# moxime/joint-vae

Hardware: AMD Instinct MI355X
Metric: training_images_per_sec (higher is better)
Workload: dtype f32

## Files before the change

include/jvae_hip.h:

```cpp
#ifndef JVAE_HIP_H
#define JVAE_HIP_H

#include <stddef.h>

#ifdef __cplusplus
extern "C" {
#endif

const char* jvae_version(void);

int jvae_gemm_f32(int M, int N, int K, int batch,
                  const float* A, long sAm, long sAk, long sAb,
                  const float* B, long sBk, long sBn, long sBb,
                  float* C, long sCm, long sCn, long sCb,
                  const float* bias, int bias_mode, int flags, int splitk, void* stream);

int jvae_splitk_fold_f32(const float* part, const float* bias, float* y, int S, long MN, int N, int relu, int accumulate,
                         void* stream);

size_t jvae_conv2d_workspace_bytes(int N, int Cin, int H, int W, int Cout, int KH, int KW, int S, int P, int OP,
                                   int transposed);
int jvae_conv2d_set_split_bf16(int mode);
int jvae_conv2d_set_split_shape16(int on);
int jvae_conv2d_out_shape(int H, int W, int KH, int KW, int S, int P, int OP, int transposed, int* OH, int* OW);
int jvae_conv2d_route(int dir, int layout, int bias, int stats, int y_f32, int aff_kind,
                      int N, int Cin, int H, int W, int Cout, int KH, int KW, int S, int P, int OP, int transposed,
                      int* kernel, int* swap, size_t* ws_bytes, int* splits, int* aff_ok);
const char* jvae_conv2d_kernel_name(int kernel);
int jvae_conv2d_fwd_f32(const float* x, const float* w, const float* bias, float* y,
                        int N, int Cin, int H, int W, int Cout, int KH, int KW, int S, int P, int OP, int transposed,
                        void* ws, size_t ws_bytes, void* stream);
int jvae_conv2d_stats_splits(int N, int Cin, int H, int W, int Cout, int KH, int KW, int S, int P, int OP, int transposed);
int jvae_conv2d_fwd_stats_f32(const float* x, const float* w, const float* bias, float* y, float* stats, int* nsplit,
                              int N, int Cin, int H, int W, int Cout, int KH, int KW, int S, int P, int OP, int transposed,
                              void* ws, size_t ws_bytes, void* stream);
int jvae_conv2d_dgrad_f32(const float* dy, const float* w, float* dx,
                          int N, int Cin, int H, int W, int Cout, int KH, int KW, int S, int P, int OP, int transposed,
                          void* ws, size_t ws_bytes, void* stream);
int jvae_conv2d_wgrad_f32(const float* x, const float* dy, float* dw, float* dbias, int accumulate,
                          int N, int Cin, int H, int W, int Cout, int KH, int KW, int S, int P, int OP, int transposed,
                          void* ws, size_t ws_bytes, void* stream);

int jvae_pack_cache_configure(void* buf, size_t bytes);
int jvae_pack_cache_begin(void* stream, long long owner, const void* const* weights, int n);
int jvae_pack_cache_end(void);
int jvae_pack_cache_pin(void);
int jvae_pack_cache_reset(void);
int jvae_pack_cache_stats(int* entries, long long* hits, long long* misses, long long* refreshes);

size_t jvae_channel_sum_workspace_bytes(int C);
int jvae_channel_sum_f32(const float* t, float* out, int N, int C, int P, int accumulate, void* ws, size_t ws_bytes,
                         void* stream);

size_t jvae_bn_workspace_bytes(int C);
int jvae_bn_plan(int N, int C, int P, int* nsplit, int* nchunk);
int jvae_image_range(int N, int parts, int j, int* nb, int* ne);
int jvae_bn_fwd_f32(const float* x, const float* gamma, const float* beta,
                    float* running_mean, float* running_var, long long* num_batches_tracked,
                    float* y, float* save_mean, float* save_invstd,
                    int N, int C, int P, float momentum, float eps, int training, int relu,
                    void* ws, size_t ws_bytes, void* stream);
int jvae_bn_fwd_ext_f32(const float* x, const float* gamma, const float* beta,
                        float* running_mean, float* running_var, long long* num_batches_tracked,
                        float* y, float* save_mean, float* save_invstd,
                        int N, int C, int P, float momentum, float eps, int training, int relu,
                        const float* ext_stats, int ext_nsplit, const float* ext_pivot,
                        void* ws, size_t ws_bytes, void* stream);
int jvae_bn_bwd_f32(const float* dy, const float* x, const float* gamma, const float* beta,
                    const float* save_mean, const float* save_invstd,
                    float* dx, float* dgamma, float* dbeta, int accumulate,
                    int N, int C, int P, int relu, void* ws, size_t ws_bytes, void* stream);
int jvae_bn_eval_bwd_f32(const float* dy, const float* x, const float* gamma, const float* beta,
                         const float* running_mean, const float* running_var, float* dx,
                         int N, int C, int P, float eps, int relu, void* stream);

int jvae_bn_finalize_f32(const float* x, const float* gamma, const float* beta,
                         float* running_mean, float* running_var, long long* num_batches_tracked,
                         float* save_mean, float* save_invstd, float* scale, float* shift,
                         int N, int C, int P, float momentum, float eps, int training,
                         const float* ext_stats, int ext_nsplit, const float* ext_pivot,
                         void* ws, size_t ws_bytes, void* stream);
int jvae_conv2d_affine_ok(int N, int Cin, int H, int W, int Cout, int KH, int KW, int S, int P, int OP, int transposed);
int jvae_conv2d_fwd_aff_f32(const float* x, const float* w, const float* bias, float* y, float* stats, int* nsplit,
                            const float* in_scale, const float* in_shift, int in_relu,
                            int N, int Cin, int H, int W, int Cout, int KH, int KW, int S, int P, int OP, int transposed,
                            void* ws, size_t ws_bytes, void* stream);
int jvae_conv2d_wgrad_aff_f32(const float* x, const float* dy, float* dw, float* dbias, int accumulate,
                              const float* in_scale, const float* in_shift, int in_relu,
                              int N, int Cin, int H, int W, int Cout, int KH, int KW, int S, int P, int OP, int transposed,
                              void* ws, size_t ws_bytes, void* stream);

int jvae_bn_sums_f32(const float* x, const float* pivot, float* sums, int N, int C, int P,
                     void* ws, size_t ws_bytes, void* stream);
int jvae_bn_fwd_sync_f32(const float* x, const float* gamma, const float* beta,
                         float* running_mean, float* running_var, long long* num_batches_tracked,
                         float* y, float* save_mean, float* save_invstd,
                         int N, int C, int P, float momentum, float eps, int relu,
                         const float* global_sums, const float* pivot, int world,
                         void* ws, size_t ws_bytes, void* stream);
int jvae_bn_bwd_sums_f32(const float* dy, const float* x, const float* gamma, const float* beta,
                         const float* save_mean, const float* save_invstd, float* local_sums,
                         int N, int C, int P, int relu, void* ws, size_t ws_bytes, void* stream);
int jvae_bn_bwd_sync_f32(const float* dy, const float* x, const float* gamma, const float* beta,
                         const float* save_mean, const float* save_invstd,
                         const float* local_sums, const float* global_sums, int world,
                         float* dx, float* dgamma, float* dbeta, int accumulate,
                         int N, int C, int P, int relu, void* stream);

int jvae_b8_pack_f32(const float* x, void* y, int N, int C, long HW, void* stream);
int jvae_b8_unpack_f32(const void* y, float* x, int N, int C, long HW, int accumulate, void* stream);
int jvae_conv2d_native_b8(int N, int Cin, int H, int W, int Cout, int KH, int KW, int S, int P, int OP, int transposed);
size_t jvae_conv2d_workspace_bytes_b8(int N, int Cin, int H, int W, int Cout, int KH, int KW, int S, int P, int OP,
                                      int transposed);
int jvae_conv2d_stats_splits_b8(int N, int Cin, int H, int W, int Cout, int KH, int KW, int S, int P, int OP, int transposed);
int jvae_conv2d_fwd_b8(const void* x, const float* w, const float* bias, void* y, int y_f32, float* stats, int* nsplit,
                       int N, int Cin, int H, int W, int Cout, int KH, int KW, int S, int P, int OP, int transposed,
                       void* ws, size_t ws_bytes, void* stream);
int jvae_conv2d_dgrad_b8(const void* dy, const float* w, void* dx,
                         int N, int Cin, int H, int W, int Cout, int KH, int KW, int S, int P, int OP, int transposed,
                         void* ws, size_t ws_bytes, void* stream);
int jvae_conv2d_wgrad_b8(const void* x, const void* dy, float* dw, float* dbias, int accumulate,
                         int N, int Cin, int H, int W, int Cout, int KH, int KW, int S, int P, int OP, int transposed,
                         void* ws, size_t ws_bytes, void* stream);
size_t jvae_bn_workspace_bytes_b8(int C);
int jvae_bn_plan_b8(int N, int C, long HW, int* nsplit, int* nchunk);
int jvae_bn_fwd_b8(const void* x, const float* gamma, const float* beta,
                   float* running_mean, float* running_var, long long* num_batches_tracked,
                   void* y, float* save_mean, float* save_invstd,
                   int N, int C, long HW, float momentum, float eps, int training, int relu,
                   const float* ext_stats, int ext_nsplit, const float* ext_pivot,
                   void* ws, size_t ws_bytes, void* stream);
int jvae_bn_bwd_b8(const void* dy, const void* x, const float* gamma, const float* beta,
                   const float* save_mean, const float* save_invstd,
                   void* dx, float* dgamma, float* dbeta, int accumulate,
                   int N, int C, long HW, int relu, void* ws, size_t ws_bytes, void* stream);
int jvae_bn_finalize_b8(const void* x, const float* gamma, const float* beta,
                        float* running_mean, float* running_var, long long* num_batches_tracked,
                        float* save_mean, float* save_invstd, float* coef,
                        int N, int C, long HW, float momentum, float eps, int training,
                        const float* ext_stats, int ext_nsplit, const float* ext_pivot,
                        void* ws, size_t ws_bytes, void* stream);
int jvae_bn_sums_b8(const void* x, const float* pivot, float* sums, int N, int C, long HW,
                    void* ws, size_t ws_bytes, void* stream);
int jvae_bn_fwd_sync_b8(const void* x, const float* gamma, const float* beta,
                        float* running_mean, float* running_var, long long* num_batches_tracked,
                        void* y, float* save_mean, float* save_invstd,
                        int N, int C, long HW, float momentum, float eps, int relu,
                        const float* global_sums, const float* pivot, int world,
                        void* ws, size_t ws_bytes, void* stream);
int jvae_bn_bwd_sums_b8(const void* dy, const void* x, const float* gamma, const float* beta,
                        const float* save_mean, const float* save_invstd, float* local_sums,
                        int N, int C, long HW, int relu, void* ws, size_t ws_bytes, void* stream);
int jvae_bn_bwd_sync_b8(const void* dy, const void* x, const float* gamma, const float* beta,
                        const float* save_mean, const float* save_invstd,
                        const float* local_sums, const float* global_sums, int world,
                        void* dx, float* dgamma, float* dbeta, int accumulate,
                        int N, int C, long HW, int relu, void* ws, size_t ws_bytes, void* stream);
int jvae_conv2d_affine_ok_b8(int N, int Cin, int H, int W, int Cout, int KH, int KW, int S, int P, int OP, int transposed);
int jvae_conv2d_fwd_aff_b8(const void* x, const float* w, const float* bias, void* y, int y_f32, float* stats, int* nsplit,
                           const float* in_scale, const float* in_shift, int in_relu,
                           int N, int Cin, int H, int W, int Cout, int KH, int KW, int S, int P, int OP, int transposed,
                           void* ws, size_t ws_bytes, void* stream);
int jvae_conv2d_wgrad_aff_b8(const void* x, const void* dy, float* dw, float* dbias, int accumulate,
                             const float* in_scale, const float* in_shift, int in_relu,
                             int N, int Cin, int H, int W, int Cout, int KH, int KW, int S, int P, int OP, int transposed,
                             void* ws, size_t ws_bytes, void* stream);
int jvae_relu_fwd_b8(const void* x, void* y, long units, void* stream);
int jvae_relu_bwd_b8(const void* dy, const void* y, void* dx, long units, void* stream);

int jvae_act_fwd_f32(const float* x, float* y, long n, int kind, void* stream);
int jvae_act_bwd_f32(const float* dy, const float* y, float* dx, long n, int kind, void* stream);

int jvae_dict_stats_f32(const float* means, float* dict, int C, int K, void* stream);
int jvae_latent_fwd_f32(const float* mu, const float* lv_raw, const float* eps, const long long* y,
                        const float* means, const float* T, const float* dict,
                        float* lv, float* z, float* kl, float* zdist, float* var_kl, float* dzdist,
                        int N, int K, int L, int C, int prior, int var_dim, float tau, float alpha, float w,
                        int sampled, int has_forced, float forced_lv, void* stream);
int jvae_latent_bwd_f32(const float* mu, const float* lv_raw, const float* lv, const float* eps, const long long* y,
                        const float* means, const float* T,
                        const float* gz, const float* g_kl, const float* g_zdist, const float* g_vkl,
                        const float* gmu_direct, const float* glv_direct,
                        float* gmu, float* glv_raw, float* gmeans, float* gT,
                        int N, int K, int L, int C, int prior, int var_dim, float tau, float alpha, float w,
                        int sampled, int has_forced, void* ws, size_t ws_bytes, void* stream);
int jvae_latent_fwd_wdev_f32(const float* mu, const float* lv_raw, const float* eps, const long long* y,
                             const float* means, const float* T, const float* dict,
                             float* lv, float* z, float* kl, float* zdist, float* var_kl, float* dzdist,
                             int N, int K, int L, int C, int prior, int var_dim, float tau, float alpha, float w,
                             int sampled, int has_forced, float forced_lv, const float* w_dev, void* stream);
int jvae_latent_bwd_wdev_f32(const float* mu, const float* lv_raw, const float* lv, const float* eps, const long long* y,
                             const float* means, const float* T,
                             const float* gz, const float* g_kl, const float* g_zdist, const float* g_vkl,
                             const float* gmu_direct, const float* glv_direct,
                             float* gmu, float* glv_raw, float* gmeans, float* gT,
                             int N, int K, int L, int C, int prior, int var_dim, float tau, float alpha, float w,
                             int sampled, int has_forced, const float* w_dev, void* ws, size_t ws_bytes, void* stream);

int jvae_recon_fwd_f32(const float* x_reco, const float* x, const float* sigma, int sigma_is_log,
                       float* wmse, int L, int N, int D, void* stream);
int jvae_recon_bwd_f32(const float* x_reco, const float* x, const float* sigma, int sigma_is_log, const float* sigma_fwd,
                       const float* g_wmse, const float* wmse, float* g_x_reco, float* gsigma, int accumulate_sigma,
                       int L, int N, int D, void* ws, size_t ws_bytes, void* stream);

int jvae_mse_rows_fwd_f32(const float* rows, const float* x, float* wmse, int L, int N, int D, void* stream);
int jvae_mse_rows_bwd_f32(const float* rows, const float* x, const float* g_wmse, float* g_rows, int L, int N, int D, void* stream);

int jvae_elbo_fwd_f32(const float* wmse_s, const float* kl, const float* ce, const float* sigma, int sigma_is_log,
                      float* wmse, float* cross_x, float* total, float* mse, int L, int N, int D, float beta, float cw,
                      void* stream);
int jvae_elbo_bwd_f32(const float* g_wmse, const float* g_cx, const float* g_tot, const float* sigma, int sigma_is_log,
                      float* g_wmse_s, float* g_kl, float* g_ce, float* gsigma, int accumulate_sigma,
                      int L, int N, int D, float beta, float cw, void* ws, size_t ws_bytes, void* stream);
int jvae_elbo_fwd_wdev_f32(const float* wmse_s, const float* kl, const float* ce, const float* sigma, int sigma_is_log,
                           float* wmse, float* cross_x, float* total, float* mse, int L, int N, int D, float beta, float cw,
                           const float* cw_dev, void* stream);
int jvae_elbo_bwd_wdev_f32(const float* g_wmse, const float* g_cx, const float* g_tot, const float* sigma, int sigma_is_log,
                           float* g_wmse_s, float* g_kl, float* g_ce, float* gsigma, int accumulate_sigma,
                           int L, int N, int D, float beta, float cw, const float* cw_dev, void* ws, size_t ws_bytes,
                           void* stream);

int jvae_dropout_f32(const float* x, float* y, long n, float p, long seed, void* stream);
int jvae_dropout_dev_f32(const float* x, float* y, long n, float p, const long long* seed_dev, long salt, void* stream);

int jvae_iws_f32(const float* wmse_s, const float* eps, const float* log_var, const float* log_pz, const float* sigma,
                 int sigma_is_log, int L, int N, int K, int C, int D, float* rows, float* iws, void* stream);

int jvae_measures_f32(const float* sumsq_x, long nx, const float* wmse, const float* zdist, const float* var_kl, int N, int Nz,
                      const float* sigma, int sigma_is_log, const float* means, int C, int K, const int* flag,
                      const float* prev, int batch, float* out, void* stream);
int jvae_measures_dev_f32(const float* sumsq_x, long nx, const float* wmse, const float* zdist, const float* var_kl, int N, int Nz,
                          const float* sigma, int sigma_is_log, const float* means, int C, int K, const int* flag,
                          float* run, int* counter, void* stream);

int jvae_loss_sums_f32(const float* const* rows, const long* lens, int nrows, float* acc, void* stream);

int jvae_xent_fwd_f32(const float* logits, const long long* y, float* ce, int R, int N, int C, void* stream);
int jvae_xent_bwd_f32(const float* logits, const long long* y, const float* g_ce, float* g_logits, int R, int N, int C,
                      void* stream);

size_t jvae_sqnorm_workspace_bytes(void);
int jvae_sqnorm_accum_f32(const float* g, long n, float* acc, int reset, void* ws, size_t ws_bytes, void* stream);
int jvae_clip_scale_f32(float* g, long n, const float* sqnorm, float max_norm, void* stream);
int jvae_adam_step_f32(float* p, const float* g, float* m, float* v, long n,
                       float lr, float beta1, float beta2, float eps, float weight_decay, long step,
                       float max_norm, const float* sqnorm, int* nonfinite_flag, void* stream);
int jvae_adam_step_dev_f32(float* p, const float* g, float* m, float* v, long n, float* hyper, int advance,
                           float eps, float weight_decay, float max_norm, const float* sqnorm, int* nonfinite_flag,
                           void* stream);

int jvae_sgd_step_f32(float* p, const float* g, float* buf, long n, float lr, float momentum, int nesterov,
                      float weight_decay, int first_step, float max_norm, const float* sqnorm, int* nonfinite_flag,
                      void* stream);

int jvae_pool2d_out_shape(int H, int W, int K, int S, int P, int* OH, int* OW);
int jvae_pool2d_fwd_f32(const float* x, float* y, int* idx, long planes, int H, int W, int K, int S, int P, int mode,
                        void* stream);
int jvae_pool2d_bwd_f32(const float* dy, const int* idx, float* dx, long planes, int H, int W, int K, int S, int P,
                        int mode, void* stream);
int jvae_upsample_nearest_fwd_f32(const float* x, float* y, long planes, int H, int W, int scale, void* stream);
int jvae_upsample_nearest_bwd_f32(const float* dy, float* dx, long planes, int H, int W, int scale, void* stream);
int jvae_pool2d_fwd_b8(const void* x, void* y, int* idx, long blocks, int H, int W, int K, int S, int P, int mode, void* stream);
int jvae_pool2d_bwd_b8(const void* dy, const int* idx, void* dx, long blocks, int H, int W, int K, int S, int P, int mode,
                       void* stream);
int jvae_upsample_nearest_fwd_b8(const void* x, void* y, long blocks, int H, int W, int scale, void* stream);
int jvae_upsample_nearest_bwd_b8(const void* dy, void* dx, long blocks, int H, int W, int scale, void* stream);

int jvae_augment_u8_f32(const unsigned char* in, const unsigned char* flip, const int* dy, const int* dx,
                        float* out, int N, int C, int H, int W, int pad, int nhwc, void* stream);

size_t jvae_roc_workspace_bytes(int M, long n_in, long n_out);
int jvae_roc_curve_f32(const float* ins, const float* outs, const double* kept_tpr, const int* two_sided,
                       double* auc, double* kept_fpr, double* kept_tpr_out, double* thr_low, double* thr_up, int* status,
                       int M, long n_in, long n_out, int K, void* ws, size_t ws_bytes, void* stream);

int jvae_misclass_scores_f32(const float* src, const int* kinds, const float* temps, const int* rows, float* out,
                             int R, int C, long N, long out_stride, void* stream);
size_t jvae_misclass_split_workspace_bytes(long N);
int jvae_misclass_split_f32(const float* scores, const unsigned char* mask, float* out, int* n_correct, int M, long N,
                            void* ws, size_t ws_bytes, void* stream);
int jvae_misclass_confusion_f32(const float* scores, const unsigned char* mask, const double* thr, int* tp, int* fp,
                                int M, long N, int K, void* stream);

int jvae_odin_head_f32(const float* logits, const float* temps, float* scores, float* dlogits,
                       int F, int L, int N, int C, long stride_f, long stride_l, void* stream);
int jvae_odin_perturb_f32(float* acc, const float* g, const float* x, const float* eps, float* out, long numel, int E,
                          void* stream);

#ifdef __cplusplus
}
#endif
#endif
```

joint-vae_amd/csrc/conv_api.hip:

```cpp
#include "common.h"
#include "jvae_internal.h"
#include "conv_dispatch.h"

namespace {

inline ConvRoute route(const ConvGeom& g, int transposed, ConvDir dir, CallFlags f = {}) {
    return jvae_conv_route(g, transposed, dir, CONV_F32, f);
}

bool affine_ok(const ConvGeom& g, int transposed, ConvDir other, const ConvRoute& r) {
    return r.aff_ok && route(g, transposed, other, {false, false, false, 1}).aff_ok;
}

int fwd_f32(const float* x, const float* w, const float* bias, float* y, float* stats, int* nsplit, const InAff* aff,
            int N, int Cin, int H, int W, int Cout, int KH, int KW, int S, int P, int OP, int transposed,
            void* ws, size_t ws_bytes, void* stream) {
    ConvGeom g; int oh, ow;
    if (nsplit) *nsplit = 0;
    if (!jvae_make_geom(N, Cin, H, W, Cout, KH, KW, S, P, OP, transposed, &g, &oh, &ow)) return JVAE_EINVAL;
    const ConvRoute r = route(g, transposed, CONV_FWD, {bias != nullptr, stats != nullptr, false, jvae_aff_kind(aff)});
    if (aff && !affine_ok(g, transposed, CONV_WGRAD, r)) return JVAE_ENOTSUP;
    if (N == 0) return 0;
    if (jvae_ws_short(r, ws, ws_bytes)) return JVAE_EWORKSPACE;
    return jvae_conv_run_fwd(r, g, x, w, bias, y, (float*)ws, ws_bytes, (hipStream_t)stream, stats, nsplit, aff);
}

int wgrad_f32(const float* x, const float* dy, float* dw, float* dbias, int accumulate, const InAff* aff,
              int N, int Cin, int H, int W, int Cout, int KH, int KW, int S, int P, int OP, int transposed,
              void* ws, size_t ws_bytes, void* stream) {
    ConvGeom g; int oh, ow;
    if (!dw || (N > 0 && (!x || !dy))) return JVAE_EINVAL;
    if (!jvae_make_geom(N, Cin, H, W, Cout, KH, KW, S, P, OP, transposed, &g, &oh, &ow)) return JVAE_EINVAL;
    const ConvRoute r = route(g, transposed, CONV_WGRAD, {false, false, false, jvae_aff_kind(aff)});
    if (aff && !affine_ok(g, transposed, CONV_FWD, r)) return JVAE_ENOTSUP;
    if (N > 0 && jvae_ws_short(r, ws, ws_bytes)) return JVAE_EWORKSPACE;
    hipStream_t st = (hipStream_t)stream;
    if (!accumulate) {
        hipError_t e = hipMemsetAsync(dw, 0, sizeof(float) * (size_t)Cin * Cout * KH * KW, st);
        if (e != hipSuccess) return (int)e;
    }
    if (N == 0) {
        if (dbias && !accumulate) {
            hipError_t e = hipMemsetAsync(dbias, 0, sizeof(float) * (size_t)Cout, st);
            if (e != hipSuccess) return (int)e;
        }
        return 0;
    }
    int rc = jvae_conv_run_wgrad(r, g, transposed, x, dy, dw, (float*)ws, ws_bytes, st, aff);
    if (rc) return rc;
    if (dbias) rc = jvae_channel_sum(dy, dbias, N, Cout, oh * ow, accumulate, (float*)ws, ws_bytes, st);
    return rc;
}

}

extern "C" {

int jvae_conv2d_set_split_bf16(int mode) { return jvae_conv5_x3_set(mode); }
int jvae_conv2d_set_split_shape16(int on) { return jvae_conv5_x3_set_shape16(on); }

size_t jvae_conv2d_workspace_bytes(int N, int Cin, int H, int W, int Cout, int KH, int KW, int S, int P, int OP,
                                   int transposed) {
    ConvGeom g; int oh, ow;
    if (!jvae_make_geom(N, Cin, H, W, Cout, KH, KW, S, P, OP, transposed, &g, &oh, &ow)) return 0;
    return jvae_conv_ws(g, transposed);
}

int jvae_conv2d_route(int dir, int layout, int bias, int stats, int y_f32, int aff_kind,
                      int N, int Cin, int H, int W, int Cout, int KH, int KW, int S, int P, int OP, int transposed,
                      int* kernel, int* swap, size_t* ws_bytes, int* splits, int* aff_ok) {
    ConvGeom g; int oh, ow;
    if (dir != CONV_FWD && dir != CONV_DGRAD && dir != CONV_WGRAD) return JVAE_EINVAL;
    if ((layout != CONV_F32 && layout != CONV_B8) || aff_kind < 0 || aff_kind > 2) return JVAE_EINVAL;
    if (!jvae_make_geom(N, Cin, H, W, Cout, KH, KW, S, P, OP, transposed, &g, &oh, &ow)) return JVAE_EINVAL;
    const ConvRoute r = jvae_conv_route(g, transposed, (ConvDir)dir, (ConvLayout)layout,
                                        {bias != 0, stats != 0, y_f32 != 0, aff_kind});
    if (kernel) *kernel = (int)r.k;
    if (swap) *swap = r.swap ? 1 : 0;
    if (ws_bytes) *ws_bytes = r.ws;
    if (splits) *splits = r.splits;
    if (aff_ok) *aff_ok = r.aff_ok ? 1 : 0;
    return 0;
}

const char* jvae_conv2d_kernel_name(int kernel) {
    switch (kernel) {
#define JVAE_CK_NAME(k) case k: return #k;
        JVAE_CK_NAME(CK_NONE) JVAE_CK_NAME(CK_GENERIC) JVAE_CK_NAME(CK_POINT) JVAE_CK_NAME(CK_SMALLCO)
        JVAE_CK_NAME(CK_SMALLCI) JVAE_CK_NAME(CK_FWD5) JVAE_CK_NAME(CK_FWD5_X3) JVAE_CK_NAME(CK_T2) JVAE_CK_NAME(CK_T2_X3)
        JVAE_CK_NAME(CK_WG5) JVAE_CK_NAME(CK_WG5_X3) JVAE_CK_NAME(CK_B8) JVAE_CK_NAME(CK_T2_B8) JVAE_CK_NAME(CK_WG_B8)
        JVAE_CK_NAME(CK_WG_B8X) JVAE_CK_NAME(CK_SMALLCO_DG)
#undef JVAE_CK_NAME
        default: return nullptr;
    }
}

int jvae_conv2d_out_shape(int H, int W, int KH, int KW, int S, int P, int OP, int transposed, int* OH, int* OW) {
    ConvGeom g;
    if (!OH || !OW) return JVAE_EINVAL;
    return jvae_make_geom(1, 1, H, W, 1, KH, KW, S, P, OP, transposed, &g, OH, OW) ? 0 : JVAE_EINVAL;
}

int jvae_conv2d_fwd_f32(const float* x, const float* w, const float* bias, float* y,
                        int N, int Cin, int H, int W, int Cout, int KH, int KW, int S, int P, int OP, int transposed,
                        void* ws, size_t ws_bytes, void* stream) {
    if (!w || (N > 0 && (!x || !y))) return JVAE_EINVAL;
    return fwd_f32(x, w, bias, y, nullptr, nullptr, nullptr, N, Cin, H, W, Cout, KH, KW, S, P, OP, transposed, ws, ws_bytes,
                   stream);
}

int jvae_conv2d_stats_splits(int N, int Cin, int H, int W, int Cout, int KH, int KW, int S, int P, int OP, int transposed) {
    ConvGeom g; int oh, ow;
    if (!jvae_make_geom(N, Cin, H, W, Cout, KH, KW, S, P, OP, transposed, &g, &oh, &ow)) return 0;
    return route(g, transposed, CONV_FWD, {false, true, false, 0}).splits;
}

int jvae_conv2d_fwd_stats_f32(const float* x, const float* w, const float* bias, float* y, float* stats, int* nsplit,
                              int N, int Cin, int H, int W, int Cout, int KH, int KW, int S, int P, int OP, int transposed,
                              void* ws, size_t ws_bytes, void* stream) {
    if (!w || !nsplit || (N > 0 && (!x || !y))) return JVAE_EINVAL;
    return fwd_f32(x, w, bias, y, stats, nsplit, nullptr, N, Cin, H, W, Cout, KH, KW, S, P, OP, transposed, ws, ws_bytes, stream);
}

int jvae_conv2d_affine_ok(int N, int Cin, int H, int W, int Cout, int KH, int KW, int S, int P, int OP, int transposed) {
    ConvGeom g; int oh, ow;
    if (!jvae_make_geom(N, Cin, H, W, Cout, KH, KW, S, P, OP, transposed, &g, &oh, &ow)) return 0;
    return affine_ok(g, transposed, CONV_WGRAD, route(g, transposed, CONV_FWD, {false, false, false, 1})) ? 1 : 0;
}

int jvae_conv2d_fwd_aff_f32(const float* x, const float* w, const float* bias, float* y, float* stats, int* nsplit,
                            const float* in_scale, const float* in_shift, int in_relu,
                            int N, int Cin, int H, int W, int Cout, int KH, int KW, int S, int P, int OP, int transposed,
                            void* ws, size_t ws_bytes, void* stream) {
    if (!w || !in_scale || !in_shift || (N > 0 && (!x || !y))) return JVAE_EINVAL;
    if (stats && !nsplit) return JVAE_EINVAL;
    const InAff aff{in_scale, in_shift, in_relu};
    return fwd_f32(x, w, bias, y, stats, nsplit, &aff, N, Cin, H, W, Cout, KH, KW, S, P, OP, transposed, ws, ws_bytes, stream);
}

int jvae_conv2d_wgrad_aff_f32(const float* x, const float* dy, float* dw, float* dbias, int accumulate,
                              const float* in_scale, const float* in_shift, int in_relu,
                              int N, int Cin, int H, int W, int Cout, int KH, int KW, int S, int P, int OP, int transposed,
                              void* ws, size_t ws_bytes, void* stream) {
    if (!in_scale || !in_shift) return JVAE_EINVAL;
    const InAff aff{in_scale, in_shift, in_relu};
    return wgrad_f32(x, dy, dw, dbias, accumulate, &aff, N, Cin, H, W, Cout, KH, KW, S, P, OP, transposed, ws, ws_bytes, stream);
}

int jvae_conv2d_dgrad_f32(const float* dy, const float* w, float* dx,
                          int N, int Cin, int H, int W, int Cout, int KH, int KW, int S, int P, int OP, int transposed,
                          void* ws, size_t ws_bytes, void* stream) {
    ConvGeom g; int oh, ow;
    if (!w || (N > 0 && (!dy || !dx))) return JVAE_EINVAL;
    if (!jvae_make_geom(N, Cin, H, W, Cout, KH, KW, S, P, OP, transposed, &g, &oh, &ow)) return JVAE_EINVAL;
    if (N == 0) return 0;
    const ConvRoute r = route(g, transposed, CONV_DGRAD);
    if (jvae_ws_short(r, ws, ws_bytes)) return JVAE_EWORKSPACE;
    return jvae_conv_run_fwd(r, g, dy, w, nullptr, dx, (float*)ws, ws_bytes, (hipStream_t)stream);
}

int jvae_conv2d_wgrad_f32(const float* x, const float* dy, float* dw, float* dbias, int accumulate,
                          int N, int Cin, int H, int W, int Cout, int KH, int KW, int S, int P, int OP, int transposed,
                          void* ws, size_t ws_bytes, void* stream) {
    return wgrad_f32(x, dy, dw, dbias, accumulate, nullptr, N, Cin, H, W, Cout, KH, KW, S, P, OP, transposed, ws, ws_bytes, stream);
}

size_t jvae_channel_sum_workspace_bytes(int C) { return jvae_channel_sum_ws_bytes(C); }

int jvae_channel_sum_f32(const float* t, float* out, int N, int C, int P, int accumulate, void* ws, size_t ws_bytes,
                         void* stream) {
    if (!t || !out || N < 0 || C <= 0 || P <= 0) return JVAE_EINVAL;
    return jvae_channel_sum(t, out, N, C, P, accumulate, (float*)ws, ws_bytes, (hipStream_t)stream);
}

}
```

joint-vae_amd/csrc/conv_dispatch.h:

```cpp
#pragma once
#include "common.h"
#include "jvae_internal.h"

size_t jvae_conv_generic_ws(const ConvGeom& g);
int jvae_fold_fwd(const ConvGeom& g, const float* xb, const float* w, const float* bias, float* ys,
                  float* ws, size_t ws_bytes, hipStream_t st);
int jvae_fold_bwd(const ConvGeom& g, const float* ys, const float* w, const float* bias, float* xb,
                  float* ws, size_t ws_bytes, hipStream_t st);
int jvae_fold_wgrad(const ConvGeom& g, const float* xb, const float* ys, float* dw,
                    float* ws, size_t ws_bytes, hipStream_t st);
size_t jvae_channel_sum_ws_bytes(int C);
int jvae_channel_sum(const float* t, float* out, int N, int C, int P, int accumulate, float* ws, size_t ws_bytes,
                     hipStream_t st);

bool jvae_conv5_fwd_ok(int Cin, int H, int W, int Cout, int OH, int OW, int S, int P);
size_t jvae_conv5_pack_floats(int Cin, int Cout);
int jvae_conv5_fwd(const float* in, const float* w, int swap, int flip, const float* bias, float* out,
                   int N, int Cin, int H, int W, int Cout, int OW, int S, int P, float* ws, hipStream_t st,
                   float* stats = nullptr, int* nsplit = nullptr, const InAff* aff = nullptr);
int jvae_conv5_fwd_max_splits(int N, int OW);

int jvae_conv5_pack(const float* w, float* wp, int C, int O, int swap, int flip, hipStream_t st);

bool jvae_conv5_x3_ok(int Cin, int H, int W, int Cout, int OH, int OW, int S, int P);
size_t jvae_conv5_x3_pack_bytes(int Cin, int Cout);
int jvae_conv5_x3_set(int mode);
int jvae_conv5_x3_set_shape16(int on);
bool jvae_conv5_x3_enabled();
int jvae_conv5_x3_wpack(const float* w, float* ws, int C, int O, int swap, int flip, hipStream_t st);
bool jvae_convt2_x3_ok(int N, int C, int WS, int O);
int jvae_convt2_x3(const float* in, const float* w, const float* bias, float* out, int N, int C, int WS, int O, float* ws,
                   hipStream_t st, float* stats = nullptr, int* nsplit = nullptr, const InAff* aff = nullptr);
int jvae_conv5_x3_fwd(const float* in, const float* w, int swap, int flip, const float* bias, float* out,
                      int N, int Cin, int H, int W, int Cout, int OW, int S, int P, float* ws, hipStream_t st,
                      float* stats = nullptr, int* nsplit = nullptr, const InAff* aff = nullptr);

bool jvae_convt2_ok(int C, int HS, int WS, int O, int HB, int WB, int KH, int KW, int S, int P);
int jvae_convt2(const float* in, const float* wpacked, const float* bias, float* out, int N, int C, int WS, int O,
                hipStream_t st, float* stats = nullptr, int* nsplit = nullptr, const InAff* aff = nullptr);

bool jvae_conv5_smallco_ok(int Cin, int H, int W, int Cout, int KH, int KW, int S, int P);
int jvae_conv5_smallco(const float* in, const float* w, const float* bias, float* out, int N, int Cin, int W, int Cout,
                       hipStream_t st, const InAff* aff = nullptr);
int jvae_conv5_smallco_dgrad(const float* dy, const float* w, float* dx, int N, int Cy, int W, int Cx, hipStream_t st);

bool jvae_conv5_smallci_ok(int Cin, int H, int W, int Cout, int OW, int S, int P, bool dgrad_role);
int jvae_conv5_smallci(const float* in, const float* w, int swap, int flip, const float* bias, float* out,
                       int N, int Cin, int W, int Cout, float* ws, hipStream_t st, float* stats = nullptr, int* nsplit = nullptr);

bool jvae_conv5_wgrad_ok(int Ca, int HS, int WS, int Cb, int HB, int WB, int S, int P);
size_t jvae_conv5_wgrad_ws_floats(int N, int Ca, int Cb, int S, int WS);
int jvae_conv5_wgrad(const float* ps, const float* q, float* dw, int accumulate, int swapflip,
                     int N, int Ca, int WS, int Cb, int S, int P, float* ws, hipStream_t st,
                     const InAff* aff_p = nullptr, const InAff* aff_q = nullptr);

bool jvae_conv5_wgrad_x3_ok(int Ca, int HS, int WS, int Cb, int HB, int WB, int S, int P);
size_t jvae_conv5_wgrad_x3_ws_floats(int N, int Ca, int Cb, int S);
int jvae_conv5_wgrad_x3(const float* ps, const float* q, float* dw, int accumulate, int swapflip,
                        int N, int Ca, int WS, int Cb, int S, int P, float* ws, hipStream_t st,
                        const InAff* aff_p = nullptr, const InAff* aff_q = nullptr);

bool jvae_make_geom(int N, int Cin, int H, int W, int Cout, int KH, int KW, int S, int P, int OP, int transposed,
                    ConvGeom* g, int* OH, int* OW);

enum ConvDir { CONV_FWD = 1, CONV_DGRAD = 2, CONV_WGRAD = 4 };
enum ConvLayout { CONV_F32, CONV_B8 };
enum ConvKernel {
    CK_NONE,
    CK_GENERIC, CK_POINT,
    CK_SMALLCO, CK_SMALLCI, CK_FWD5, CK_FWD5_X3, CK_T2, CK_T2_X3, CK_WG5, CK_WG5_X3,
    CK_B8, CK_T2_B8, CK_WG_B8, CK_WG_B8X,
    CK_SMALLCO_DG,
};
struct CallFlags {
    bool bias, stats;
    bool y_f32;
    int aff;
};
struct ConvRoute {
    ConvKernel k;
    bool swap;
    int S, P;
    size_t ws;
    int splits;
    bool aff_ok;
};
ConvRoute jvae_conv_route(const ConvGeom& g, int transposed, ConvDir dir, ConvLayout layout, CallFlags f);
inline int jvae_aff_kind(const InAff* aff) { return !aff ? 0 : (aff->relu == JVAE_ACT_LEAKY ? 2 : 1); }
inline bool jvae_ws_short(const ConvRoute& r, const void* ws, size_t ws_bytes) { return r.ws && (!ws || ws_bytes < r.ws); }
template <class T>
inline void jvae_wgrad_operands(const ConvRoute& r, int transposed, T* x, T* dy, const InAff* aff, T** ps, T** q,
                                const InAff** aff_p, const InAff** aff_q) {
    const bool p_is_x = r.swap != (transposed != 0);
    *ps = p_is_x ? x : dy;
    *q = p_is_x ? dy : x;
    *aff_p = p_is_x ? aff : nullptr;
    *aff_q = p_is_x ? nullptr : aff;
}

size_t jvae_conv_ws(const ConvGeom& g, int transposed);
int jvae_conv_run_fwd(const ConvRoute& r, const ConvGeom& g, const float* in, const float* w, const float* bias, float* out,
                      float* ws, size_t ws_bytes, hipStream_t st, float* stats = nullptr, int* nsplit = nullptr,
                      const InAff* aff = nullptr);
int jvae_conv_run_wgrad(const ConvRoute& r, const ConvGeom& g, int transposed, const float* x, const float* dy, float* dw,
                        float* ws, size_t ws_bytes, hipStream_t st, const InAff* aff = nullptr);
```

joint-vae_amd/csrc/conv_dispatch.hip:

```cpp
#include "common.h"
#include "conv_dispatch.h"
#include "conv_b8.h"
#include "pack_elems.h"

namespace {

inline bool is5(const ConvGeom& g) { return g.KH == 5 && g.KW == 5; }
inline bool is3p1(const ConvGeom& g) { return g.KH == 3 && g.KW == 3 && g.P == 1; }
inline size_t max_sz(size_t a, size_t b) { return a > b ? a : b; }

inline bool point_input(const ConvGeom& g) {
    return g.Hs == 1 && g.Ws == 1 && g.P == 0 && g.S == 1 && g.Hb == g.KH && g.Wb == g.KW;
}
inline int point_wgrad_pieces(const ConvGeom& g) {
    const int want = (int)(1024 / ((long)cdiv(g.Cs, 64) * cdiv(g.Cb * g.KH * g.KW, 64)));
    return want < 1 ? 1 : (want > 8 ? 8 : want);
}

struct FwdOp { int Ci, H, W, Co, OH, OW; };
inline FwdOp fwd_op(const ConvGeom& g, bool small_in) {
    return small_in ? FwdOp{g.Cs, g.Hs, g.Ws, g.Cb, g.Hb, g.Wb} : FwdOp{g.Cb, g.Hb, g.Wb, g.Cs, g.Hs, g.Ws};
}
struct WgOp { int Ca, HS, WS, Cb, HB, WB; };
inline WgOp wg_op(const ConvGeom& g, bool swap) {
    return swap ? WgOp{g.Cb, g.Hb, g.Wb, g.Cs, g.Hs, g.Ws} : WgOp{g.Cs, g.Hs, g.Ws, g.Cb, g.Hb, g.Wb};
}

inline bool b8_aff_ok(int Cin, const CallFlags& f) { return (Cin + 7) / 8 * 8 <= 256 && f.aff != 2; }

ConvRoute fwd_route(const ConvGeom& g, int transposed, ConvDir dir, bool b8, const CallFlags& f) {
    const bool small_in = (dir == CONV_FWD) == (transposed != 0);
    const FwdOp o = fwd_op(g, small_in);
    ConvRoute r{CK_NONE, small_in, small_in ? 1 : g.S, small_in ? g.KH - 1 - g.P : g.P, 0, 0, false};
    if (!b8 && transposed && point_input(g)) {
        r.k = CK_POINT;
        if (!small_in) r.ws = 4 * (size_t)16 * g.N * g.Cs;
        return r;
    }
    if (!b8 && dir == CONV_FWD && !transposed && jvae_conv5_smallco_ok(g.Cb, g.Hb, g.Wb, g.Cs, g.KH, g.KW, g.S, g.P)) {
        r.k = CK_SMALLCO;
        r.aff_ok = g.Cb <= 256;
        return r;
    }
    if (!b8 && dir == CONV_DGRAD && !transposed && g.Hs == g.Hb && g.Ws == g.Wb &&
        jvae_conv5_smallco_ok(g.Cs, g.Hb, g.Wb, g.Cb, g.KH, g.KW, g.S, g.P)) {
        r.k = CK_SMALLCO_DG;
        return r;
    }
    if (small_in && g.S == 2) {
        if (b8 && jvae_convt2_b8_ok(g.Cs, g.Hs, g.Ws, g.Cb, g.Hb, g.Wb, g.KH, g.KW, g.S, g.P) && !f.y_f32) {
            r = ConvRoute{CK_T2_B8, true, 2, g.P, jvae_conv5_b8_pack_bytes(g.Cs, g.Cb, g.KH), jvae_conv5_b8_max_splits(g.N, g.Ws),
                          b8_aff_ok(g.Cs, f)};
        } else if (!b8 && jvae_convt2_ok(g.Cs, g.Hs, g.Ws, g.Cb, g.Hb, g.Wb, g.KH, g.KW, g.S, g.P)) {
            r = ConvRoute{jvae_convt2_x3_ok(g.N, g.Cs, g.Ws, g.Cb) ? CK_T2_X3 : CK_T2, true, 2, g.P,
                          4 * jvae_conv5_pack_floats(g.Cs, g.Cb), jvae_conv5_fwd_max_splits(g.N, g.Ws), true};
        }
    } else if ((is5(g) || (b8 && is3p1(g))) && (!small_in || g.S == 1)) {
        if (b8 && jvae_conv5_b8_fwd_ok(o.Ci, o.H, o.W, o.Co, o.OH, o.OW, r.S, r.P, g.KH)) {
            r.k = CK_B8;
            r.ws = jvae_conv5_b8_pack_bytes(o.Ci, o.Co, g.KH);
            r.splits = jvae_conv5_b8_max_splits(g.N, o.OW);
            r.aff_ok = b8_aff_ok(o.Ci, f);
        } else if (!b8 && jvae_conv5_fwd_ok(o.Ci, o.H, o.W, o.Co, o.OH, o.OW, r.S, r.P)) {
            if (jvae_conv5_x3_ok(o.Ci, o.H, o.W, o.Co, o.OW, o.OW, r.S, r.P)) r.k = CK_FWD5_X3;
            else if (!f.aff && jvae_conv5_smallci_ok(o.Ci, o.H, o.W, o.Co, o.OW, r.S, r.P, !f.bias && !f.stats)) r.k = CK_SMALLCI;
            else r.k = CK_FWD5;
            r.ws = 4 * jvae_conv5_pack_floats(o.Ci, o.Co);
            r.splits = jvae_conv5_fwd_max_splits(g.N, o.OW);
            r.aff_ok = true;
        }
    }
    if (r.k == CK_NONE && !b8) r = ConvRoute{CK_GENERIC, small_in, g.S, g.P, 0, 0, false};
    return r;
}

ConvRoute wgrad_route(const ConvGeom& g, int transposed, bool b8, const CallFlags& f) {
    const int few = b8 ? 8 : 15;
    const bool swap = g.S == 1 && g.Cs <= few && g.Cb > few && g.Hs == g.Hb;
    const WgOp o = wg_op(g, swap);
    ConvRoute r{CK_NONE, swap, swap ? 1 : g.S, swap ? g.KH - 1 - g.P : g.P, 0, 0, false};
    if ((is5(g) || is3p1(g)) && b8 && jvae_conv5_wgrad_b8_ok(o.Ca, o.HS, o.WS, o.Cb, o.HB, o.WB, r.S, r.P, g.KH)) {
        const bool x = is5(g) && jvae_conv5_wgrad_b8x_ok(o.Ca, o.WS, o.WS, o.Cb, o.WS * r.S, o.WS * r.S, r.S, r.P);
        r.k = x ? CK_WG_B8X : CK_WG_B8;
        r.ws = 4 * jvae_conv5_wgrad_b8_ws_floats(g.N, o.Ca, o.Cb, g.KH);
        r.aff_ok = f.aff != 2;
    } else if (is5(g) && !b8 && jvae_conv5_wgrad_ok(o.Ca, o.HS, o.WS, o.Cb, o.HB, o.WB, r.S, r.P)) {
        const bool x = jvae_conv5_wgrad_x3_ok(o.Ca, o.WS, o.WS, o.Cb, o.WS * r.S, o.WS * r.S, r.S, r.P);
        r.k = x ? CK_WG5_X3 : CK_WG5;
        r.ws = 4 * jvae_conv5_wgrad_ws_floats(g.N, o.Ca, o.Cb, r.S, o.WS);
        r.aff_ok = true;
    } else if (!b8 && transposed && point_input(g)) {
        r.k = CK_POINT;
        r.ws = 4 * (size_t)point_wgrad_pieces(g) * g.Cs * g.Cb * g.KH * g.KW;
    } else if (!b8) {
        r.k = CK_GENERIC;
    }
    return r;
}

inline const float* packed_f32(const float* w, float* ws, int C, int O, int swap, int flip, hipStream_t st) {
    bool fresh = true;
    float* slot = (float*)jvae_pack_cache_get(JVAE_PACK_F32, w, C, O, swap, flip, &fresh);
    if (slot && fresh) return slot;
    float* dst = slot ? slot : ws;
    return jvae_conv5_pack(w, dst, C, O, swap, flip, st) == 0 ? dst : nullptr;
}

}

bool jvae_make_geom(int N, int Cin, int H, int W, int Cout, int KH, int KW, int S, int P, int OP, int transposed,
                    ConvGeom* g, int* OH, int* OW) {
    if (N < 0 || Cin <= 0 || Cout <= 0 || H <= 0 || W <= 0 || KH <= 0 || KW <= 0 || S <= 0 || P < 0 || OP < 0)
        return false;
    g->N = N; g->KH = KH; g->KW = KW; g->S = S; g->P = P;
    if (!transposed) {
        if (OP != 0) return false;
        *OH = (H + 2 * P - KH) / S + 1;
        *OW = (W + 2 * P - KW) / S + 1;
        g->Cb = Cin; g->Hb = H; g->Wb = W;
        g->Cs = Cout; g->Hs = *OH; g->Ws = *OW;
    } else {
        if (OP >= S && OP != 0) return false;
        *OH = (H - 1) * S - 2 * P + KH + OP;
        *OW = (W - 1) * S - 2 * P + KW + OP;
        g->Cs = Cin; g->Hs = H; g->Ws = W;
        g->Cb = Cout; g->Hb = *OH; g->Wb = *OW;
    }
    return *OH > 0 && *OW > 0;
}

ConvRoute jvae_conv_route(const ConvGeom& g, int transposed, ConvDir dir, ConvLayout layout, CallFlags f) {
    if (dir == CONV_WGRAD) return wgrad_route(g, transposed, layout == CONV_B8, f);
    return fwd_route(g, transposed, dir, layout == CONV_B8, f);
}

size_t jvae_conv_ws(const ConvGeom& g, int transposed) {
    size_t a = max_sz(jvae_conv_generic_ws(g), jvae_channel_sum_ws_bytes(g.Cb > g.Cs ? g.Cb : g.Cs));
    for (ConvDir d : {CONV_FWD, CONV_DGRAD, CONV_WGRAD}) a = max_sz(a, jvae_conv_route(g, transposed, d, CONV_F32, {}).ws);
    if (is5(g)) a = max_sz(a, 4 * jvae_conv5_pack_floats(g.Cb, g.Cs));
    if (transposed && point_input(g)) a = max_sz(a, 4 * (size_t)8 * g.Cs * g.Cb * g.KH * g.KW);
    return a;
}

int jvae_conv_run_fwd(const ConvRoute& r, const ConvGeom& g, const float* in, const float* w, const float* bias, float* out,
                      float* ws, size_t ws_bytes, hipStream_t st, float* stats, int* nsplit, const InAff* aff) {
    const FwdOp o = fwd_op(g, r.swap);
    const int sw = r.swap ? 1 : 0;
    switch (r.k) {
        case CK_SMALLCO: return jvae_conv5_smallco(in, w, bias, out, g.N, g.Cb, g.Wb, g.Cs, st, aff);
        case CK_SMALLCO_DG: return jvae_conv5_smallco_dgrad(in, w, out, g.N, g.Cs, g.Wb, g.Cb, st);
        case CK_SMALLCI: return jvae_conv5_smallci(in, w, sw, sw, bias, out, g.N, o.Ci, o.W, o.Co, ws, st, stats, nsplit);
        case CK_FWD5_X3:
            return jvae_conv5_x3_fwd(in, w, sw, sw, bias, out, g.N, o.Ci, o.H, o.W, o.Co, o.OW, r.S, r.P, ws, st, stats, nsplit, aff);
        case CK_FWD5:
            return jvae_conv5_fwd(in, w, sw, sw, bias, out, g.N, o.Ci, o.H, o.W, o.Co, o.OW, r.S, r.P, ws, st, stats, nsplit, aff);
        case CK_T2_X3: return jvae_convt2_x3(in, w, bias, out, g.N, g.Cs, g.Ws, g.Cb, ws, st, stats, nsplit, aff);
        case CK_T2: {
            const float* wp = packed_f32(w, ws, g.Cs, g.Cb, 1, 0, st);
            if (!wp) return JVAE_EINVAL;
            return jvae_convt2(in, wp, bias, out, g.N, g.Cs, g.Ws, g.Cb, st, stats, nsplit, aff);
        }
        case CK_POINT: {
            const int cols = g.Cb * g.KH * g.KW;
            if (r.swap)
                return jvae_gemm_launch_ex(g.N, cols, g.Cs, 1, in, g.Cs, 1, 0, w, cols, 1, 0, out, cols, 1, 0,
                                           bias, bias ? 1 : 0, g.KH * g.KW, 0, 1, st);
            const long outf = (long)g.N * g.Cs;
            int S = 0;
            int rc = jvae_gemm_launch_part(g.N, g.Cs, cols, 1, in, cols, 1, 0, w, 1, cols, 0, ws, g.Cs, 1, 0, outf, 16, &S, st);
            if (rc) return rc;
            return jvae_splitk_fold(ws, nullptr, out, S, outf, g.Cs, 0, 0, st);
        }
        case CK_GENERIC:
            return r.swap ? jvae_fold_bwd(g, in, w, bias, out, ws, ws_bytes, st) : jvae_fold_fwd(g, in, w, bias, out, ws, ws_bytes, st);
        default: return JVAE_ENOTSUP;
    }
}

int jvae_conv_run_wgrad(const ConvRoute& r, const ConvGeom& g, int transposed, const float* x, const float* dy, float* dw,
                        float* ws, size_t ws_bytes, hipStream_t st, const InAff* aff) {
    const float *ps, *q;
    const InAff *aff_p, *aff_q;
    jvae_wgrad_operands(r, transposed, x, dy, aff, &ps, &q, &aff_p, &aff_q);
    const WgOp o = wg_op(g, r.swap);
    const float* big = transposed ? dy : x;
    const float* small = transposed ? x : dy;
    switch (r.k) {
        case CK_WG5_X3:
            return jvae_conv5_wgrad_x3(ps, q, dw, 1, r.swap, g.N, o.Ca, o.WS, o.Cb, r.S, r.P, ws, st,
                                       aff_p, aff_q);
        case CK_WG5:
            return jvae_conv5_wgrad(ps, q, dw, 1, r.swap, g.N, o.Ca, o.WS, o.Cb, r.S, r.P, ws, st,
                                    aff_p, aff_q);
        case CK_POINT: {
            const int cols = g.Cb * g.KH * g.KW;
            const long outf = (long)g.Cs * cols;
            int S = 0;
            int rc = jvae_gemm_launch_part(g.Cs, cols, g.N, 1, small, 1, g.Cs, 0, big, cols, 1, 0, ws, cols, 1, 0, outf,
                                           point_wgrad_pieces(g), &S, st);
            if (rc) return rc;
            return jvae_splitk_fold(ws, nullptr, dw, S, outf, cols, 0, 1, st);
        }
        case CK_GENERIC: return jvae_fold_wgrad(g, big, small, dw, ws, ws_bytes, st);
        default: return JVAE_ENOTSUP;
    }
}
```

joint-vae_amd/csrc/conv_generic.hip:

```cpp
#include "common.h"
#include "jvae_internal.h"

namespace {

__global__ __launch_bounds__(256) void unfold_kernel(const float* __restrict__ xb, float* __restrict__ col,
                                                     ConvGeom g, int n0, int nimg, long sn, long sk, long sq,
                                                     int kfast) {
    const int Kd = g.Cb * g.KH * g.KW, Ps = g.Hs * g.Ws;
    const long total = (long)nimg * Kd * Ps;
    for (long i = (long)blockIdx.x * blockDim.x + threadIdx.x; i < total; i += (long)gridDim.x * blockDim.x) {
        int n, k, q;
        if (kfast) { k = (int)(i % Kd); long r = i / Kd; n = (int)(r % nimg); q = (int)(r / nimg); }
        else       { q = (int)(i % Ps); long r = i / Ps; k = (int)(r % Kd);  n = (int)(r / Kd); }
        const int kw = k % g.KW, kh = (k / g.KW) % g.KH, cb = k / (g.KW * g.KH);
        const int hs = q / g.Ws, ws = q % g.Ws;
        const int hb = hs * g.S + kh - g.P, wb = ws * g.S + kw - g.P;
        float v = 0.f;
        if (hb >= 0 && hb < g.Hb && wb >= 0 && wb < g.Wb)
            v = xb[(((long)(n0 + n) * g.Cb + cb) * g.Hb + hb) * g.Wb + wb];
        col[(long)n * sn + (long)k * sk + (long)q * sq] = v;
    }
}

template <bool KFAST>
__global__ __launch_bounds__(256) void unfold4_kernel(const float* __restrict__ xb, float* __restrict__ col,
                                                      ConvGeom g, int n0, int nimg) {
    const unsigned Kd = g.Cb * g.KH * g.KW, Ps = g.Hs * g.Ws, KK = g.KH * g.KW;
    const unsigned inner4 = (KFAST ? Kd : Ps) / 4;
    const unsigned total = (KFAST ? Ps * (unsigned)nimg : (unsigned)nimg * Kd) * inner4;
    for (unsigned i = blockIdx.x * blockDim.x + threadIdx.x; i < total; i += gridDim.x * blockDim.x) {
        const unsigned row = i / inner4, e4 = (i - row * inner4) * 4;
        unsigned n, k, q;
        if (KFAST) { q = row / nimg; n = row - q * nimg; k = e4; }
        else       { n = row / Kd;   k = row - n * Kd;   q = e4; }
        unsigned cb = k / KK, t = k - cb * KK;
        unsigned kh = t / g.KW, kw = t - kh * g.KW;
        const unsigned hs = q / g.Ws, ws = q - hs * g.Ws;
        const float* src = xb + (long)(n0 + n) * g.Cb * g.Hb * g.Wb;
        f32x4 v;
#pragma unroll
        for (int e = 0; e < 4; ++e) {
            const int hb = (int)(hs * g.S + kh) - g.P;
            const int wb = (int)((KFAST ? ws : ws + e) * g.S + kw) - g.P;
            v[e] = (hb >= 0 && hb < g.Hb && wb >= 0 && wb < g.Wb) ? src[((long)cb * g.Hb + hb) * g.Wb + wb] : 0.f;
            if (KFAST && ++kw == (unsigned)g.KW) { kw = 0; if (++kh == (unsigned)g.KH) { kh = 0; ++cb; } }
        }
        *reinterpret_cast<f32x4*>(col + (long)i * 4) = v;
    }
}

__global__ __launch_bounds__(256) void fold_kernel(const float* __restrict__ col, float* __restrict__ xb,
                                                   const float* __restrict__ bias, ConvGeom g, int n0, int nimg,
                                                   long sn, long sk, long sq) {
    const unsigned total = (unsigned)nimg * g.Cb * g.Hb * g.Wb;
    for (unsigned i = blockIdx.x * blockDim.x + threadIdx.x; i < total; i += gridDim.x * blockDim.x) {
        unsigned r = i / (unsigned)g.Wb;
        const int wb = (int)(i - r * g.Wb);
        unsigned r2 = r / (unsigned)g.Hb;
        const int hb = (int)(r - r2 * g.Hb);
        const int n = (int)(r2 / (unsigned)g.Cb);
        const int cb = (int)(r2 - (unsigned)n * g.Cb);
        float acc = bias ? bias[cb] : 0.f;
        if (g.Hs * g.Ws < g.KH * g.KW) {
            for (int hs = 0; hs < g.Hs; ++hs) {
                const int kh = hb + g.P - hs * g.S;
                if (kh < 0 || kh >= g.KH) continue;
                for (int ws = 0; ws < g.Ws; ++ws) {
                    const int kw = wb + g.P - ws * g.S;
                    if (kw < 0 || kw >= g.KW) continue;
                    const int k = (cb * g.KH + kh) * g.KW + kw;
                    acc += col[(long)n * sn + (long)k * sk + (long)(hs * g.Ws + ws) * sq];
                }
            }
            xb[(((long)(n0 + n) * g.Cb + cb) * g.Hb + hb) * g.Wb + wb] = acc;
            continue;
        }
        for (int kh = 0; kh < g.KH; ++kh) {
            const int th = hb + g.P - kh;
            if (th < 0 || th % g.S) continue;
            const int hs = th / g.S;
            if (hs >= g.Hs) continue;
            for (int kw = 0; kw < g.KW; ++kw) {
                const int tw = wb + g.P - kw;
                if (tw < 0 || tw % g.S) continue;
                const int ws = tw / g.S;
                if (ws >= g.Ws) continue;
                const int k = (cb * g.KH + kh) * g.KW + kw;
                acc += col[(long)n * sn + (long)k * sk + (long)(hs * g.Ws + ws) * sq];
            }
        }
        xb[(((long)(n0 + n) * g.Cb + cb) * g.Hb + hb) * g.Wb + wb] = acc;
    }
}

__global__ __launch_bounds__(256) void channel_sum_kernel(const float* __restrict__ t, float* __restrict__ partial,
                                                          int N, int C, int P, int nsplit) {
    __shared__ float red[17];
    const int c = blockIdx.x, sp = blockIdx.y;
    const ImageRange ir = image_range(N, nsplit, sp);
    const int nb = ir.nb, ne = ir.ne;
    float s = 0.f;
    if ((P & 3) == 0) {
        const int P4 = P >> 2;
        const long cnt = (long)(ne - nb) * P4;
        for (long i = threadIdx.x; i < cnt; i += blockDim.x) {
            const long n = nb + i / P4, q = i % P4;
            const f32x4 v = *reinterpret_cast<const f32x4*>(t + (n * C + c) * (long)P + q * 4);
            s += (v[0] + v[1]) + (v[2] + v[3]);
        }
    } else {
        const long cnt = (long)(ne - nb) * P;
        for (long i = threadIdx.x; i < cnt; i += blockDim.x) {
            const long n = nb + i / P, q = i % P;
            s += t[(n * C + c) * (long)P + q];
        }
    }
    s = block_sum(s, red);
    if (threadIdx.x == 0) partial[(long)c * nsplit + sp] = s;
}

__global__ void channel_fold_kernel(const float* __restrict__ partial, float* __restrict__ out, int C, int nsplit,
                                    int accumulate) {
    const int c = blockIdx.x * blockDim.x + threadIdx.x;
    if (c >= C) return;
    float s = 0.f;
    for (int k = 0; k < nsplit; ++k) s += partial[(long)c * nsplit + k];
    out[c] = (accumulate ? out[c] : 0.f) + s;
}

inline int fold_slab_images(const ConvGeom& g) {
    const long per = (long)g.Cb * g.Hb * g.Wb;
    long n = ((1L << 31) - 1) / (per > 0 ? per : 1);
    if (const char* e = getenv("JVAE_FOLD_SLAB")) { const long v = atol(e); if (v > 0 && v < n) n = v; }
    return (int)(n < 1 ? 1 : (n > g.N ? (g.N > 0 ? g.N : 1) : n));
}

inline int grid_for(long total) {
    long b = (total + 255) / 256;
    return (int)(b > 8192 ? 8192 : (b < 1 ? 1 : b));
}

inline int grid_for4(long total4) {
    long b = (total4 + 255) / 256;
    return (int)(b > 16384 ? 16384 : (b < 1 ? 1 : b));
}

int launch_unfold(const float* xb, float* col, const ConvGeom& g, int n0, int nimg, bool kfast, hipStream_t st) {
    const long Kd = (long)g.Cb * g.KH * g.KW, Ps = (long)g.Hs * g.Ws, total = (long)nimg * Kd * Ps;
    const bool vec = total < (1L << 31) && (kfast ? Kd % 4 == 0 : g.Ws % 4 == 0) && ((uintptr_t)col & 15) == 0;
    if (vec && kfast)
        hipLaunchKernelGGL(unfold4_kernel<true>, dim3(grid_for4(total / 4)), dim3(256), 0, st, xb, col, g, n0, nimg);
    else if (vec)
        hipLaunchKernelGGL(unfold4_kernel<false>, dim3(grid_for4(total / 4)), dim3(256), 0, st, xb, col, g, n0, nimg);
    else if (kfast)
        hipLaunchKernelGGL(unfold_kernel, dim3(grid_for(total)), dim3(256), 0, st, xb, col, g, n0, nimg, Kd, 1L, (long)nimg * Kd, 1);
    else
        hipLaunchKernelGGL(unfold_kernel, dim3(grid_for(total)), dim3(256), 0, st, xb, col, g, n0, nimg, Kd * Ps, Ps, 1L, 0);
    JVAE_LAUNCH_CHECK();
    return 0;
}

inline bool pixel_batched(const ConvGeom& g) { return g.Hs * g.Ws <= 48; }

inline bool wgrad_joint(const ConvGeom& g) { return pixel_batched(g) && g.Hs * g.Ws > 1; }
inline int wgrad_slices(const ConvGeom& g) {
    const long Kd = (long)g.Cb * g.KH * g.KW, K = (long)g.Hs * g.Ws * g.N;
    const long tiles = (long)cdiv(g.Cs, 64) * cdiv(Kd, 64);
    for (int S = 16; S > 1; S >>= 1)
        if (tiles * S <= 2048 && K % S == 0 && K / S >= 256) return S;
    return 1;
}

inline int fwd_slices(const ConvGeom& g) {
    if (!pixel_batched(g)) return 1;
    const long Kd = (long)g.Cb * g.KH * g.KW;
    const long tiles = (long)cdiv(g.N, 64) * cdiv(g.Cs, 64) * g.Hs * g.Ws;
    if (tiles < 1 || tiles >= 512 || Kd < 1024) return 1;
    int s = (int)(1024 / tiles);
    return s > 8 ? 8 : (s < 1 ? 1 : s);
}

__global__ __launch_bounds__(256) void small_transpose_kernel(const float* __restrict__ ys, float* __restrict__ yt,
                                                              int N, int Cs, int Ps) {
    const long total = (long)N * Cs * Ps;
    for (long i = (long)blockIdx.x * blockDim.x + threadIdx.x; i < total; i += (long)gridDim.x * blockDim.x) {
        const int cs = (int)(i % Cs);
        const long r = i / Cs;
        const int n = (int)(r % N), q = (int)(r / N);
        yt[i] = ys[((long)n * Cs + cs) * Ps + q];
    }
}

inline long col_floats_per_image(const ConvGeom& g) { return (long)g.Cb * g.KH * g.KW * g.Hs * g.Ws; }

inline long wgrad_part_floats(const ConvGeom& g) { return (long)g.Cs * g.Cb * g.KH * g.KW; }

}

size_t jvae_conv_generic_ws(const ConvGeom& g) {
    const long per = (col_floats_per_image(g) + (pixel_batched(g) ? 0 : wgrad_part_floats(g))) * 4;
    long imgs = (1L << 30) / (per > 0 ? per : 1);
    if (imgs < 1) imgs = 1;
    if (imgs > g.N) imgs = g.N;
    if (pixel_batched(g)) imgs = g.N;
    size_t bytes = (size_t)(imgs * per);
    size_t extra = 0;
    if (wgrad_joint(g))
        extra = 4 * ((size_t)g.N * g.Cs * g.Hs * g.Ws + (size_t)wgrad_slices(g) * g.Cs * g.Cb * g.KH * g.KW);
    const size_t fwd_extra = fwd_slices(g) > 1 ? 4 * (size_t)fwd_slices(g) * g.N * g.Cs * g.Hs * g.Ws : 0;
    return bytes + (extra > fwd_extra ? extra : fwd_extra);
}

static int chunk_images(const ConvGeom& g, size_t ws_bytes) {
    const long per = col_floats_per_image(g) * 4;
    long imgs = (long)(ws_bytes / (size_t)(per > 0 ? per : 1));
    if (imgs > g.N) imgs = g.N;
    return (int)imgs;
}

int jvae_fold_fwd(const ConvGeom& g, const float* xb, const float* w, const float* bias, float* ys,
                  float* ws, size_t ws_bytes, hipStream_t st) {
    const int Kd = g.Cb * g.KH * g.KW, Ps = g.Hs * g.Ws;
    if (pixel_batched(g)) {
        if (ws_bytes < (size_t)col_floats_per_image(g) * 4 * g.N) return JVAE_EWORKSPACE;
        { const int rc = launch_unfold(xb, ws, g, 0, g.N, true, st); if (rc) return rc; }
        const int want = fwd_slices(g);
        if (want > 1) {
            const long colf = (long)col_floats_per_image(g) * g.N, outf = (long)g.N * g.Cs * Ps;
            if (ws_bytes < 4 * (size_t)(colf + want * outf)) return JVAE_EWORKSPACE;
            float* part = ws + colf;
            int S = 0;
            int rc = jvae_gemm_launch_part(g.N, g.Cs, Kd, Ps, ws, Kd, 1, (long)g.N * Kd, w, 1, Kd, 0,
                                           part, g.Cs, 1, (long)g.N * g.Cs, outf, want, &S, st);
            if (rc) return rc;
            return jvae_splitk_fold_qn(part, bias, ys, S, g.N, g.Cs, Ps, st);
        }
        return jvae_gemm_launch(g.N, g.Cs, Kd, Ps, ws, Kd, 1, (long)g.N * Kd, w, 1, Kd, 0,
                                ys, (long)g.Cs * Ps, Ps, 1, bias, bias ? 1 : 0, 0, 1, st);
    }
    const int chunk = chunk_images(g, ws_bytes);
    if (chunk < 1) return JVAE_EWORKSPACE;
    for (int n0 = 0; n0 < g.N; n0 += chunk) {
        const int ni = (g.N - n0 < chunk) ? g.N - n0 : chunk;
        { const int rc = launch_unfold(xb, ws, g, n0, ni, false, st); if (rc) return rc; }
        int rc = jvae_gemm_launch(g.Cs, Ps, Kd, ni, w, Kd, 1, 0, ws, Ps, 1, (long)Kd * Ps,
                                  ys + (long)n0 * g.Cs * Ps, Ps, 1, (long)g.Cs * Ps, bias, bias ? 2 : 0, 0, 1, st);
        if (rc) return rc;
    }
    return 0;
}

int jvae_fold_bwd(const ConvGeom& g, const float* ys, const float* w, const float* bias, float* xb,
                  float* ws, size_t ws_bytes, hipStream_t st) {
    const int Kd = g.Cb * g.KH * g.KW, Ps = g.Hs * g.Ws;
    if (pixel_batched(g)) {
        if (ws_bytes < (size_t)col_floats_per_image(g) * 4 * g.N) return JVAE_EWORKSPACE;
        const long colf = (long)col_floats_per_image(g) * g.N, ytf = (long)g.N * g.Cs * Ps;
        int rc;
        if (Ps > 1 && ws_bytes >= 4 * (size_t)(colf + ytf)) {
            float* yt = ws + colf;
            hipLaunchKernelGGL(small_transpose_kernel, dim3(grid_for(ytf)), dim3(256), 0, st, ys, yt, g.N, g.Cs, Ps);
            JVAE_LAUNCH_CHECK();
            rc = jvae_gemm_launch(g.N, Kd, g.Cs, Ps, yt, g.Cs, 1, (long)g.N * g.Cs, w, Kd, 1, 0,
                                  ws, Kd, 1, (long)g.N * Kd, nullptr, 0, 0, 1, st);
        } else {
            rc = jvae_gemm_launch(g.N, Kd, g.Cs, Ps, ys, (long)g.Cs * Ps, Ps, 1, w, Kd, 1, 0,
                                  ws, Kd, 1, (long)g.N * Kd, nullptr, 0, 0, 1, st);
        }
        if (rc) return rc;
        const int slab = fold_slab_images(g);
        for (int n0 = 0; n0 < g.N; n0 += slab) {
            const int ni = (g.N - n0 < slab) ? g.N - n0 : slab;
            hipLaunchKernelGGL(fold_kernel, dim3(grid_for((long)ni * g.Cb * g.Hb * g.Wb)), dim3(256), 0, st,
                               ws + (long)n0 * Kd, xb, bias, g, n0, ni, (long)Kd, 1L, (long)g.N * Kd);
            JVAE_LAUNCH_CHECK();
        }
        return 0;
    }
    const int chunk = chunk_images(g, ws_bytes);
    if (chunk < 1) return JVAE_EWORKSPACE;
    for (int n0 = 0; n0 < g.N; n0 += chunk) {
        const int ni = (g.N - n0 < chunk) ? g.N - n0 : chunk;
        int rc = jvae_gemm_launch(Kd, Ps, g.Cs, ni, w, 1, Kd, 0, ys + (long)n0 * g.Cs * Ps, Ps, 1, (long)g.Cs * Ps,
                                  ws, Ps, 1, (long)Kd * Ps, nullptr, 0, 0, 1, st);
        if (rc) return rc;
        const int slab = fold_slab_images(g);
        for (int m0 = 0; m0 < ni; m0 += slab) {
            const int mi = (ni - m0 < slab) ? ni - m0 : slab;
            hipLaunchKernelGGL(fold_kernel, dim3(grid_for((long)mi * g.Cb * g.Hb * g.Wb)), dim3(256), 0, st,
                               ws + (long)m0 * Kd * Ps, xb, bias, g, n0 + m0, mi, (long)Kd * Ps, (long)Ps, 1L);
            JVAE_LAUNCH_CHECK();
        }
    }
    return 0;
}

int jvae_fold_wgrad(const ConvGeom& g, const float* xb, const float* ys, float* dw,
                    float* ws, size_t ws_bytes, hipStream_t st) {
    const int Kd = g.Cb * g.KH * g.KW, Ps = g.Hs * g.Ws;
    if (pixel_batched(g)) {
        if (ws_bytes < (size_t)col_floats_per_image(g) * 4 * g.N) return JVAE_EWORKSPACE;
        { const int rc = launch_unfold(xb, ws, g, 0, g.N, true, st); if (rc) return rc; }
        if (wgrad_joint(g)) {
            const int S = wgrad_slices(g);
            const long colf = (long)col_floats_per_image(g) * g.N, ytf = (long)g.N * g.Cs * Ps;
            if (ws_bytes < 4 * (size_t)(colf + ytf + (long)S * g.Cs * Kd)) return JVAE_EWORKSPACE;
            float* yt = ws + colf;
            float* part = yt + ytf;
            hipLaunchKernelGGL(small_transpose_kernel, dim3(grid_for(ytf)), dim3(256), 0, st, ys, yt, g.N, g.Cs, Ps);
            JVAE_LAUNCH_CHECK();
            const long Ks = (long)Ps * g.N / S;
            int rc = jvae_gemm_launch(g.Cs, Kd, (int)Ks, S, yt, 1, g.Cs, Ks * g.Cs, ws, Kd, 1, Ks * Kd,
                                      part, Kd, 1, (long)g.Cs * Kd, nullptr, 0, 0, 1, st);
            if (rc) return rc;
            return jvae_splitk_fold(part, nullptr, dw, S, (long)g.Cs * Kd, Kd, 0, 1, st);
        }
        for (int q = 0; q < Ps; ++q) {
            int rc = jvae_gemm_launch(g.Cs, Kd, g.N, 1, ys + q, Ps, (long)g.Cs * Ps, 0, ws + (long)q * g.N * Kd, Kd, 1, 0,
                                      dw, Kd, 1, 0, nullptr, 0, 1, 1, st);
            if (rc) return rc;
        }
        return 0;
    }
    const long colf = col_floats_per_image(g), partf = wgrad_part_floats(g);
    long chunk = (long)(ws_bytes / (size_t)(4 * (colf + partf)));
    if (chunk > g.N) chunk = g.N;
    if (chunk < 1) {
        if (chunk_images(g, ws_bytes) < 1) return JVAE_EWORKSPACE;
        chunk = 1;
    }
    float* part = ws + chunk * colf;
    for (int n0 = 0; n0 < g.N; n0 += (int)chunk) {
        const int ni = (g.N - n0 < chunk) ? g.N - n0 : (int)chunk;
        { const int rc = launch_unfold(xb, ws, g, n0, ni, false, st); if (rc) return rc; }
        const float* a = ys + (long)n0 * g.Cs * Ps;
        if (ni == 1) {
            const int rc = jvae_gemm_launch(g.Cs, Kd, Ps, 1, a, Ps, 1, 0, ws, 1, Ps, 0, dw, Kd, 1, 0, nullptr, 0, 1, 1, st);
            if (rc) return rc;
            continue;
        }
        int rc = jvae_gemm_launch(g.Cs, Kd, Ps, ni, a, Ps, 1, (long)g.Cs * Ps, ws, 1, Ps, (long)Kd * Ps,
                                  part, Kd, 1, partf, nullptr, 0, 0, 1, st);
        if (rc) return rc;
        rc = jvae_splitk_fold(part, nullptr, dw, ni, partf, Kd, 0, 1, st);
        if (rc) return rc;
    }
    return 0;
}

size_t jvae_channel_sum_ws_bytes(int C) { return sizeof(float) * (size_t)(C > 0 ? C : 1) * 64; }

int jvae_channel_sum(const float* t, float* out, int N, int C, int P, int accumulate, float* ws, size_t ws_bytes,
                     hipStream_t st) {
    if (C <= 0) return 0;
    if (N <= 0) {
        if (!accumulate) {
            hipError_t e = hipMemsetAsync(out, 0, sizeof(float) * (size_t)C, st);
            if (e != hipSuccess) return (int)e;
        }
        return 0;
    }
    if (!ws || ws_bytes < jvae_channel_sum_ws_bytes(C)) return JVAE_EWORKSPACE;
    long work = (long)N * P;
    int ns = (int)(work / 4096);
    const int cap = (1024 + C - 1) / C;
    if (ns > cap) ns = cap;
    if (ns > 64) ns = 64;
    if (ns > N) ns = N;
    if (ns < 1) ns = 1;
    hipLaunchKernelGGL(channel_sum_kernel, dim3(C, ns), dim3(256), 0, st, t, ws, N, C, P, ns);
    JVAE_LAUNCH_CHECK();
    hipLaunchKernelGGL(channel_fold_kernel, dim3(cdiv(C, 64)), dim3(64), 0, st, (const float*)ws, out, C, ns, accumulate);
    JVAE_LAUNCH_CHECK();
    return 0;
}
```

joint-vae_amd/csrc/gemm.hip:

```cpp
#include <stdlib.h>
#include "common.h"
#include "conv_x3.h"
#include "jvae_internal.h"
#include "conv_dispatch.h"

namespace {

constexpr int BK = 32;
constexpr int KQ = BK / 4;

struct GemmP {
    const float* A; long sAm, sAk, sAb;
    const float* B; long sBk, sBn, sBb;
    float* C; long sCm, sCn, sCb;
    const float* bias;
    int bias_mode;
    int bias_div;
    int M, N, K;
    int splitk;
    int kchunk;
    int flags;
    long sCsplit;
    int vecA, vecB;
    int xcd;
};

template <bool VEC>
__device__ __forceinline__ f32x4 load4(const float* p, long stride, int i0, int lim, bool row_ok) {
    f32x4 v = {0.f, 0.f, 0.f, 0.f};
    if (!row_ok) return v;
    if (VEC) {
        if (i0 + 3 < lim) return *reinterpret_cast<const f32x4*>(p);
    }
#pragma unroll
    for (int j = 0; j < 4; ++j)
        if (i0 + j < lim) v[j] = p[j * stride];
    return v;
}

template <int BM, int BN, bool AK, bool BNC>
__global__ __launch_bounds__(256) void gemm_kernel(GemmP p) {
    constexpr int LDA = BM + 4, LDB = BN + 4;
    constexpr int WM = BM / 2, WN = BN / 2;
    constexpr int TM = WM / 32, TN = WN / 32;
    constexpr int GA = BM * BK / 4 / 256;
    constexpr int GB = BN * BK / 4 / 256;
    __shared__ float As[BK * LDA];
    __shared__ float Bs[BK * LDB];

    const int tid = threadIdx.x, lane = tid & 63, wave = tid >> 6;
    const int wm0 = (wave >> 1) * WM, wn0 = (wave & 1) * WN;
    const int m0 = blockIdx.y * BM, n0 = blockIdx.x * BN;
    const int batch = blockIdx.z / p.splitk, split = blockIdx.z % p.splitk;
    const int kbeg = split * p.kchunk;
    const int kend = min(p.K, kbeg + p.kchunk);
    const float* A = p.A + (long)batch * p.sAb;
    const float* B = p.B + (long)batch * p.sBb;
    float* C = p.C + (long)batch * p.sCb + ((p.flags & 8) ? (long)split * p.sCsplit : 0L);

    f32x16 acc[TM][TN];
#pragma unroll
    for (int i = 0; i < TM; ++i)
#pragma unroll
        for (int j = 0; j < TN; ++j)
#pragma unroll
            for (int r = 0; r < 16; ++r) acc[i][j][r] = 0.f;

    f32x4 ra[GA], rb[GB];

    auto gload = [&](int k0) {
#pragma unroll
        for (int g = 0; g < GA; ++g) {
            if (AK) {
                const int kq = tid % KQ, row = tid / KQ + g * (256 / KQ);
                const int m = m0 + row, k = k0 + kq * 4;
                const float* src = A + (long)m * p.sAm + (long)k * p.sAk;
                ra[g] = p.vecA ? load4<true>(src, p.sAk, k, kend, m < p.M) : load4<false>(src, p.sAk, k, kend, m < p.M);
            } else {
                constexpr int GPR = BM / 4;
                const int mq = tid % GPR, kr = tid / GPR + g * (256 / GPR);
                const int m = m0 + mq * 4, k = k0 + kr;
                const float* src = A + (long)m * p.sAm + (long)k * p.sAk;
                ra[g] = p.vecA ? load4<true>(src, p.sAm, m, p.M, k < kend) : load4<false>(src, p.sAm, m, p.M, k < kend);
            }
        }
#pragma unroll
        for (int g = 0; g < GB; ++g) {
            if (BNC) {
                constexpr int GPR = BN / 4;
                const int nq = tid % GPR, kr = tid / GPR + g * (256 / GPR);
                const int n = n0 + nq * 4, k = k0 + kr;
                const float* src = B + (long)k * p.sBk + (long)n * p.sBn;
                rb[g] = p.vecB ? load4<true>(src, p.sBn, n, p.N, k < kend) : load4<false>(src, p.sBn, n, p.N, k < kend);
            } else {
                const int kq = tid % KQ, col = tid / KQ + g * (256 / KQ);
                const int n = n0 + col, k = k0 + kq * 4;
                const float* src = B + (long)k * p.sBk + (long)n * p.sBn;
                rb[g] = p.vecB ? load4<true>(src, p.sBk, k, kend, n < p.N) : load4<false>(src, p.sBk, k, kend, n < p.N);
            }
        }
    };
    auto lstore = [&]() {
#pragma unroll
        for (int g = 0; g < GA; ++g) {
            if (AK) {
                const int kq = tid % KQ, row = tid / KQ + g * (256 / KQ);
#pragma unroll
                for (int j = 0; j < 4; ++j) As[(kq * 4 + j) * LDA + row] = ra[g][j];
            } else {
                constexpr int GPR = BM / 4;
                const int mq = tid % GPR, kr = tid / GPR + g * (256 / GPR);
                *reinterpret_cast<f32x4*>(&As[kr * LDA + mq * 4]) = ra[g];
            }
        }
#pragma unroll
        for (int g = 0; g < GB; ++g) {
            if (BNC) {
                constexpr int GPR = BN / 4;
                const int nq = tid % GPR, kr = tid / GPR + g * (256 / GPR);
                *reinterpret_cast<f32x4*>(&Bs[kr * LDB + nq * 4]) = rb[g];
            } else {
                const int kq = tid % KQ, col = tid / KQ + g * (256 / KQ);
#pragma unroll
                for (int j = 0; j < 4; ++j) Bs[(kq * 4 + j) * LDB + col] = rb[g][j];
            }
        }
    };

    const int half = lane >> 5, l31 = lane & 31;
    if (kbeg < kend) gload(kbeg);
    for (int k0 = kbeg; k0 < kend; k0 += BK) {
        __syncthreads();
        lstore();
        __syncthreads();
        if (k0 + BK < kend) gload(k0 + BK);
#pragma unroll
        for (int kk = 0; kk < BK / 2; ++kk) {
            float a[TM], b[TN];
#pragma unroll
            for (int i = 0; i < TM; ++i) a[i] = As[(2 * kk + half) * LDA + wm0 + i * 32 + l31];
#pragma unroll
            for (int j = 0; j < TN; ++j) b[j] = Bs[(2 * kk + half) * LDB + wn0 + j * 32 + l31];
#pragma unroll
            for (int i = 0; i < TM; ++i)
#pragma unroll
                for (int j = 0; j < TN; ++j)
                    acc[i][j] = __builtin_amdgcn_mfma_f32_32x32x2f32(a[i], b[j], acc[i][j], 0, 0, 0);
        }
    }

    const bool lead = (split == 0) && !(p.flags & 8);
#pragma unroll
    for (int i = 0; i < TM; ++i)
#pragma unroll
        for (int j = 0; j < TN; ++j) {
            const int n = n0 + wn0 + j * 32 + l31;
            if (n >= p.N) continue;
            float bn = (p.bias_mode == 1 && lead) ? p.bias[n / p.bias_div] : 0.f;
#pragma unroll
            for (int r = 0; r < 16; ++r) {
                const int m = m0 + wm0 + i * 32 + (r & 3) + 8 * (r >> 2) + 4 * half;
                if (m >= p.M) continue;
                float v = acc[i][j][r] + bn;
                if (p.bias_mode == 2 && lead) v += p.bias[m];
                float* dst = C + (long)m * p.sCm + (long)n * p.sCn;
                if (p.flags & 8) {
                    *dst = v;
                } else if (p.flags & 4) {
                    atomicAdd(dst, v);
                } else {
                    if (p.flags & 1) v += *dst;
                    if (p.flags & 2) v = fmaxf(v, 0.f);
                    *dst = v;
                }
            }
        }
}

template <int BM, int BN>
int launch_tile(const GemmP& p, int batch, hipStream_t st) {
    dim3 grid(cdiv(p.N, BN), cdiv(p.M, BM), batch * p.splitk), block(256);
    const bool ak = (p.sAk == 1), bnc = (p.sBn == 1);
    if (ak && bnc)       hipLaunchKernelGGL((gemm_kernel<BM, BN, true, true>), grid, block, 0, st, p);
    else if (ak && !bnc) hipLaunchKernelGGL((gemm_kernel<BM, BN, true, false>), grid, block, 0, st, p);
    else if (!ak && bnc) hipLaunchKernelGGL((gemm_kernel<BM, BN, false, true>), grid, block, 0, st, p);
    else                 hipLaunchKernelGGL((gemm_kernel<BM, BN, false, false>), grid, block, 0, st, p);
    JVAE_LAUNCH_CHECK();
    return 0;
}

inline bool aligned16(const void* p) { return (reinterpret_cast<uintptr_t>(p) & 15) == 0; }

typedef __bf16 gx_bf16x8 __attribute__((ext_vector_type(8)));
typedef __bf16 gx_bf16x4 __attribute__((ext_vector_type(4)));
typedef unsigned int gx_u32x2 __attribute__((ext_vector_type(2)));
typedef unsigned int gx_u32x4 __attribute__((ext_vector_type(4)));
typedef __attribute__((address_space(3))) gx_bf16x4 gx_lds_bf16x4;
constexpr int BKX = 32;

__device__ __forceinline__ void gx_split4(const f32x4& v, gx_u32x2 (&out)[3]) {
#pragma unroll
    for (int j = 0; j < 2; ++j) {
        unsigned h, m, l;
        x3_split2(x3_f32x2{v[2 * j], v[2 * j + 1]}, h, m, l);
        out[0][j] = h; out[1][j] = m; out[2][j] = l;
    }
}

template <bool KC>
struct GxImg {
    static constexpr int PITCH = KC ? (BKX * 2 + 16) : (64 * 2 + 64);
    static constexpr int ROWS = KC ? 64 : BKX;
    static constexpr int BYTES = PITCH * ROWS;
};

template <bool AK, bool BNC, int DEPTH = 1>
__global__ __launch_bounds__(256, 4) void gemm_x3_kernel(GemmP p) {
    using IA = GxImg<AK>;
    using IB = GxImg<!BNC>;
    constexpr int BM = 64, BN = 64, G4 = BM * BKX / 4 / 256;
    constexpr int KQX = BKX / 4;
    extern __shared__ __attribute__((aligned(16))) unsigned char gx_lds[];
    unsigned char* As = gx_lds;
    unsigned char* Bs = gx_lds + 3 * IA::BYTES;

    const int tid = threadIdx.x, lane = tid & 63, wave = tid >> 6;
    const int half = lane >> 5, l31 = lane & 31;
    const int cg = (lane >> 4) & 1, q4 = (lane & 15) >> 2, pp = lane & 3;
    const int wm0 = (wave >> 1) * 32, wn0 = (wave & 1) * 32;
    unsigned bx = blockIdx.x, by = blockIdx.y, bz = blockIdx.z;
    if (p.xcd) {
        const unsigned lin = (unsigned)xcd_tile(bx + gridDim.x * (by + gridDim.y * bz), gridDim.x * gridDim.y * gridDim.z);
        bx = lin % gridDim.x; by = (lin / gridDim.x) % gridDim.y; bz = lin / (gridDim.x * gridDim.y);
    }
    const int m0 = by * BM, n0 = bx * BN;
    const int batch = bz / p.splitk, split = bz % p.splitk;
    const int kbeg = split * p.kchunk;
    const int kend = min(p.K, kbeg + p.kchunk);
    const float* A = p.A + (long)batch * p.sAb;
    const float* B = p.B + (long)batch * p.sBb;
    float* C = p.C + (long)batch * p.sCb + ((p.flags & 8) ? (long)split * p.sCsplit : 0L);

    f32x16 acc;
#pragma unroll
    for (int r = 0; r < 16; ++r) acc[r] = 0.f;
    f32x4 ra[DEPTH][G4], rb[DEPTH][G4];

    auto coordA = [&](int g, int k0, int* fast, int* slow) {
        if (AK) { *fast = k0 + (tid % KQX) * 4; *slow = m0 + tid / KQX + g * (256 / KQX); }
        else    { *fast = m0 + (tid % 16) * 4;  *slow = k0 + tid / 16 + g * 16; }
    };
    auto coordB = [&](int g, int k0, int* fast, int* slow) {
        if (BNC) { *fast = n0 + (tid % 16) * 4;  *slow = k0 + tid / 16 + g * 16; }
        else     { *fast = k0 + (tid % KQX) * 4; *slow = n0 + tid / KQX + g * (256 / KQX); }
    };
    auto okA = [&](int fast, int slow) { return AK ? (fast < kend && slow < p.M) : (fast + 3 < p.M && slow < kend); };
    auto okB = [&](int fast, int slow) { return BNC ? (fast + 3 < p.N && slow < kend) : (fast < kend && slow < p.N); };

    auto gload = [&](int st, int k0) {
#pragma unroll
        for (int g = 0; g < G4; ++g) {
            if constexpr (DEPTH > 1) {
                int f, sl;
                coordA(g, k0, &f, &sl);
                const float* sa = AK ? A + (long)sl * p.sAm + f : A + (long)sl * p.sAk + f;
                ra[st][g] = *reinterpret_cast<const f32x4*>(okA(f, sl) ? sa : A);
                coordB(g, k0, &f, &sl);
                const float* sb = BNC ? B + (long)sl * p.sBk + f : B + (long)sl * p.sBn + f;
                rb[st][g] = *reinterpret_cast<const f32x4*>(okB(f, sl) ? sb : B);
                continue;
            }
            if (AK) {
                const int kq = tid % KQX, row = tid / KQX + g * (256 / KQX);
                const int m = m0 + row, k = k0 + kq * 4;
                const float* src = A + (long)m * p.sAm + (long)k * p.sAk;
                ra[st][g] = p.vecA ? load4<true>(src, p.sAk, k, kend, m < p.M) : load4<false>(src, p.sAk, k, kend, m < p.M);
            } else {
                const int mq = tid % 16, kr = tid / 16 + g * 16;
                const int m = m0 + mq * 4, k = k0 + kr;
                const float* src = A + (long)m * p.sAm + (long)k * p.sAk;
                ra[st][g] = p.vecA ? load4<true>(src, p.sAm, m, p.M, k < kend) : load4<false>(src, p.sAm, m, p.M, k < kend);
            }
            if (BNC) {
                const int nq = tid % 16, kr = tid / 16 + g * 16;
                const int n = n0 + nq * 4, k = k0 + kr;
                const float* src = B + (long)k * p.sBk + (long)n * p.sBn;
                rb[st][g] = p.vecB ? load4<true>(src, p.sBn, n, p.N, k < kend) : load4<false>(src, p.sBn, n, p.N, k < kend);
            } else {
                const int kq = tid % KQX, col = tid / KQX + g * (256 / KQX);
                const int n = n0 + col, k = k0 + kq * 4;
                const float* src = B + (long)k * p.sBk + (long)n * p.sBn;
                rb[st][g] = p.vecB ? load4<true>(src, p.sBk, k, kend, n < p.N) : load4<false>(src, p.sBk, k, kend, n < p.N);
            }
        }
    };
    auto lstore = [&](int st, int k0) {
#pragma unroll
        for (int g = 0; g < G4; ++g) {
            const int fa = AK ? tid % KQX : tid % 16, sa_ = AK ? tid / KQX + g * (256 / KQX) : tid / 16 + g * 16;
            const int fb = BNC ? tid % 16 : tid % KQX, sb_ = BNC ? tid / 16 + g * 16 : tid / KQX + g * (256 / KQX);
            f32x4 va = ra[st][g], vb = rb[st][g];
            if constexpr (DEPTH > 1) {
                int f, sl;
                coordA(g, k0, &f, &sl);
                if (!okA(f, sl)) va = f32x4{0.f, 0.f, 0.f, 0.f};
                coordB(g, k0, &f, &sl);
                if (!okB(f, sl)) vb = f32x4{0.f, 0.f, 0.f, 0.f};
            }
            gx_u32x2 sa[3], sb[3];
            gx_split4(va, sa);
            gx_split4(vb, sb);
#pragma unroll
            for (int pl = 0; pl < 3; ++pl) {
                *reinterpret_cast<gx_u32x2*>(As + pl * IA::BYTES + sa_ * IA::PITCH + fa * 8) = sa[pl];
                *reinterpret_cast<gx_u32x2*>(Bs + pl * IB::BYTES + sb_ * IB::PITCH + fb * 8) = sb[pl];
            }
        }
    };
    auto frag = [&](const unsigned char* img, bool kc, int pitch, int r0, int ks) -> gx_bf16x8 {
        if (kc)
            return __builtin_bit_cast(gx_bf16x8, *reinterpret_cast<const gx_u32x4*>(img + (r0 + l31) * pitch + (ks * 16 + half * 8) * 2));
        const unsigned char* q = img + (ks * 16 + half * 8 + q4) * pitch + (r0 + cg * 16 + pp * 4) * 2;
        const gx_bf16x4 lo = __builtin_amdgcn_ds_read_tr16_b64_v4bf16((gx_lds_bf16x4*)q);
        const gx_bf16x4 hi = __builtin_amdgcn_ds_read_tr16_b64_v4bf16((gx_lds_bf16x4*)(q + 4 * pitch));
        return __builtin_shufflevector(lo, hi, 0, 1, 2, 3, 4, 5, 6, 7);
    };

    auto multiply = [&]() {
#pragma unroll
        for (int ks = 0; ks < BKX / 16; ++ks) {
            gx_bf16x8 a[3], b[3];
#pragma unroll
            for (int pl = 0; pl < 3; ++pl) {
                a[pl] = frag(As + pl * IA::BYTES, AK, IA::PITCH, wm0, ks);
                b[pl] = frag(Bs + pl * IB::BYTES, !BNC, IB::PITCH, wn0, ks);
            }
            constexpr int APL[6] = {0, 2, 1, 0, 1, 0}, BPL[6] = {2, 0, 1, 1, 0, 0};
#pragma unroll
            for (int t = 0; t < 6; ++t) acc = __builtin_amdgcn_mfma_f32_32x32x16_bf16(a[APL[t]], b[BPL[t]], acc, 0, 0, 0);
        }
    };
    if constexpr (DEPTH > 1) {
#pragma unroll
        for (int d = 0; d < DEPTH; ++d) gload(d, kbeg + d * BKX);
        const int nst = (kend - kbeg + BKX - 1) / BKX;
        int k0 = kbeg;
        for (int it = 0; it < nst / DEPTH; ++it, k0 += DEPTH * BKX) {
#pragma unroll
            for (int d = 0; d < DEPTH; ++d) {
                const int kk = k0 + d * BKX;
                __syncthreads();
                lstore(d, kk);
                __syncthreads();
                gload(d, kk + DEPTH * BKX);
                multiply();
            }
        }
#pragma unroll
        for (int d = 0; d < DEPTH - 1; ++d) {
            const int kk = k0 + d * BKX;
            if (kk < kend) {
                __syncthreads();
                lstore(d, kk);
                __syncthreads();
                multiply();
            }
        }
    } else {
        if (kbeg < kend) gload(0, kbeg);
        for (int k0 = kbeg; k0 < kend; k0 += BKX) {
            __syncthreads();
            lstore(0, k0);
            __syncthreads();
            if (k0 + BKX < kend) gload(0, k0 + BKX);
            multiply();
        }
    }

    const bool lead = (split == 0) && !(p.flags & 8);
    const int n = n0 + wn0 + l31;
    if (n >= p.N) return;
    const float bn = (p.bias_mode == 1 && lead) ? p.bias[n / p.bias_div] : 0.f;
#pragma unroll
    for (int r = 0; r < 16; ++r) {
        const int m = m0 + wm0 + (r & 3) + 8 * (r >> 2) + 4 * half;
        if (m >= p.M) continue;
        float v = acc[r] + bn;
        if (p.bias_mode == 2 && lead) v += p.bias[m];
        float* dst = C + (long)m * p.sCm + (long)n * p.sCn;
        if (p.flags & 8) {
            *dst = v;
        } else if (p.flags & 4) {
            atomicAdd(dst, v);
        } else {
            if (p.flags & 1) v += *dst;
            if (p.flags & 2) v = fmaxf(v, 0.f);
            *dst = v;
        }
    }
}

template <bool AK, bool BNC, int DEPTH>
int launch_x3_variant(const GemmP& p, int batch, hipStream_t st) {
    constexpr int LDS = 3 * (GxImg<AK>::BYTES + GxImg<!BNC>::BYTES);
    static bool attr_set = false;
    if (!attr_set) {
        hipError_t e = hipFuncSetAttribute(reinterpret_cast<const void*>(&gemm_x3_kernel<AK, BNC, DEPTH>),
                                           hipFuncAttributeMaxDynamicSharedMemorySize, LDS);
        if (e != hipSuccess) return (int)e;
        attr_set = true;
    }
    dim3 grid(cdiv(p.N, 64), cdiv(p.M, 64), batch * p.splitk), block(256);
    hipLaunchKernelGGL((gemm_x3_kernel<AK, BNC, DEPTH>), grid, block, LDS, st, p);
    JVAE_LAUNCH_CHECK();
    return 0;
}

template <bool AK, bool BNC>
int launch_x3_ab(const GemmP& p, int batch, hipStream_t st) {
    const bool deep = p.vecA && p.vecB && p.K % 4 == 0
                      && (AK || p.M % 4 == 0) && (!BNC || p.N % 4 == 0);
    if (deep) return launch_x3_variant<AK, BNC, 3>(p, batch, st);
    return launch_x3_variant<AK, BNC, 1>(p, batch, st);
}

int launch_x3(const GemmP& p0, int batch, hipStream_t st) {
    GemmP p = p0;
    p.xcd = 1;
    const bool ak = (p.sAk == 1), bnc = (p.sBn == 1);
    if (ak && bnc) return launch_x3_ab<true, true>(p, batch, st);
    if (ak) return launch_x3_ab<true, false>(p, batch, st);
    if (bnc) return launch_x3_ab<false, true>(p, batch, st);
    return launch_x3_ab<false, false>(p, batch, st);
}

inline bool gemm_x3_on(int K) {
    return K >= 64 && jvae_conv5_x3_enabled();
}

}

int jvae_gemm_launch(int M, int N, int K, int batch,
                     const float* A, long sAm, long sAk, long sAb,
                     const float* B, long sBk, long sBn, long sBb,
                     float* C, long sCm, long sCn, long sCb,
                     const float* bias, int bias_mode, int flags, int splitk, hipStream_t st) {
    return jvae_gemm_launch_ex(M, N, K, batch, A, sAm, sAk, sAb, B, sBk, sBn, sBb, C, sCm, sCn, sCb, bias, bias_mode, 1,
                               flags, splitk, st);
}

int jvae_gemm_launch_ex(int M, int N, int K, int batch,
                        const float* A, long sAm, long sAk, long sAb,
                        const float* B, long sBk, long sBn, long sBb,
                        float* C, long sCm, long sCn, long sCb,
                        const float* bias, int bias_mode, int bias_div, int flags, int splitk, hipStream_t st) {
    if (M <= 0 || N <= 0 || batch <= 0) return 0;
    if (K < 0 || !A || !B || !C) return JVAE_EINVAL;
    if (bias_mode && !bias) return JVAE_EINVAL;
    GemmP p;
    p.A = A; p.sAm = sAm; p.sAk = sAk; p.sAb = sAb;
    p.B = B; p.sBk = sBk; p.sBn = sBn; p.sBb = sBb;
    p.C = C; p.sCm = sCm; p.sCn = sCn; p.sCb = sCb;
    p.bias = bias; p.bias_mode = bias_mode; p.bias_div = bias_div > 0 ? bias_div : 1;
    p.M = M; p.N = N; p.K = K;
    if (splitk < 1) splitk = 1;
    int ktiles = cdiv(K, BK);
    if (splitk > ktiles) splitk = ktiles > 0 ? ktiles : 1;
    p.kchunk = cdiv(ktiles, splitk) * BK;
    splitk = K > 0 ? cdiv(K, p.kchunk) : 1;
    p.splitk = splitk;
    p.flags = flags & ~8;
    p.sCsplit = 0;
    if (splitk > 1) {
        if (flags & 2) return JVAE_EINVAL;
        p.flags |= 4;
    }
    const bool ak = (sAk == 1), bnc = (sBn == 1);
    p.vecA = aligned16(A) && (sAb % 4 == 0) && (ak ? (sAm % 4 == 0) : (sAm == 1 && sAk % 4 == 0));
    p.vecB = aligned16(B) && (sBb % 4 == 0) && (bnc ? (sBk % 4 == 0) : (sBk == 1 && sBn % 4 == 0));
    if (gemm_x3_on(K)) return launch_x3(p, batch, st);
    const long tiles128 = (long)cdiv(M, 128) * cdiv(N, 128) * batch * splitk;
    if (M > 64 && N > 64 && tiles128 >= 512) return launch_tile<128, 128>(p, batch, st);
    return launch_tile<64, 64>(p, batch, st);
}

int jvae_gemm_launch_part(int M, int N, int K, int batch,
                          const float* A, long sAm, long sAk, long sAb,
                          const float* B, long sBk, long sBn, long sBb,
                          float* part, long sCm, long sCn, long sCb, long sCsplit, int want_splits, int* splits,
                          hipStream_t st) {
    if (splits) *splits = 0;
    if (M <= 0 || N <= 0 || batch <= 0) return 0;
    if (K <= 0 || !A || !B || !part || !splits) return JVAE_EINVAL;
    GemmP p;
    p.A = A; p.sAm = sAm; p.sAk = sAk; p.sAb = sAb;
    p.B = B; p.sBk = sBk; p.sBn = sBn; p.sBb = sBb;
    p.C = part; p.sCm = sCm; p.sCn = sCn; p.sCb = sCb;
    p.bias = nullptr; p.bias_mode = 0; p.bias_div = 1;
    p.M = M; p.N = N; p.K = K;
    int splitk = want_splits < 1 ? 1 : want_splits;
    const int ktiles = cdiv(K, BK);
    if (splitk > ktiles) splitk = ktiles;
    p.kchunk = cdiv(ktiles, splitk) * BK;
    splitk = cdiv(K, p.kchunk);
    p.splitk = splitk;
    p.flags = 8;
    p.sCsplit = sCsplit;
    const bool ak = (sAk == 1), bnc = (sBn == 1);
    p.vecA = aligned16(A) && (sAb % 4 == 0) && (ak ? (sAm % 4 == 0) : (sAm == 1 && sAk % 4 == 0));
    p.vecB = aligned16(B) && (sBb % 4 == 0) && (bnc ? (sBk % 4 == 0) : (sBk == 1 && sBn % 4 == 0));
    *splits = splitk;
    if (gemm_x3_on(K)) return launch_x3(p, batch, st);
    return launch_tile<64, 64>(p, batch, st);
}

__global__ __launch_bounds__(256) void splitk_fold_kernel(const float* __restrict__ part, const float* __restrict__ bias,
                                                          float* __restrict__ y, int S, long MN, int N, int relu,
                                                          int accumulate, int bias_div) {
    for (long i = (long)blockIdx.x * blockDim.x + threadIdx.x; i < MN; i += (long)gridDim.x * blockDim.x) {
        float v = bias ? bias[(i / bias_div) % N] : 0.f;
        for (int s = 0; s < S; ++s) v += part[(long)s * MN + i];
        if (accumulate) v += y[i];
        y[i] = relu ? fmaxf(v, 0.f) : v;
    }
}

__global__ __launch_bounds__(256) void splitk_fold_qn_kernel(const float* __restrict__ part, const float* __restrict__ bias,
                                                             float* __restrict__ y, int S, int N, int Cs, int Ps) {
    const long total = (long)Ps * N * Cs;
    for (long i = (long)blockIdx.x * blockDim.x + threadIdx.x; i < total; i += (long)gridDim.x * blockDim.x) {
        const int cs = (int)(i % Cs);
        const long r = i / Cs;
        const int n = (int)(r % N), q = (int)(r / N);
        float v = bias ? bias[cs] : 0.f;
        for (int s = 0; s < S; ++s) v += part[(long)s * total + i];
        y[((long)n * Cs + cs) * Ps + q] = v;
    }
}

int jvae_splitk_fold_qn(const float* part, const float* bias, float* y, int S, int N, int Cs, int Ps, hipStream_t st) {
    const long total = (long)Ps * N * Cs;
    if (total == 0) return 0;
    const int blocks = (int)((total + 255) / 256 > 4096 ? 4096 : (total + 255) / 256);
    hipLaunchKernelGGL(splitk_fold_qn_kernel, dim3(blocks), dim3(256), 0, st, part, bias, y, S, N, Cs, Ps);
    JVAE_LAUNCH_CHECK();
    return 0;
}

int jvae_splitk_fold(const float* part, const float* bias, float* y, int S, long MN, int N, int relu, int accumulate,
                     hipStream_t st, int bias_div) {
    if (MN == 0) return 0;
    const int blocks = (int)((MN + 255) / 256 > 4096 ? 4096 : (MN + 255) / 256);
    hipLaunchKernelGGL(splitk_fold_kernel, dim3(blocks), dim3(256), 0, st, part, bias, y, S, MN, N, relu, accumulate,
                       bias_div > 0 ? bias_div : 1);
    JVAE_LAUNCH_CHECK();
    return 0;
}

extern "C" int jvae_splitk_fold_f32(const float* part, const float* bias, float* y, int S, long MN, int N, int relu,
                                    int accumulate, void* stream) {
    if (!part || !y || S < 1 || MN < 0 || N < 1) return JVAE_EINVAL;
    return jvae_splitk_fold(part, bias, y, S, MN, N, relu, accumulate, (hipStream_t)stream);
}

extern "C" int jvae_gemm_f32(int M, int N, int K, int batch,
                             const float* A, long sAm, long sAk, long sAb,
                             const float* B, long sBk, long sBn, long sBb,
                             float* C, long sCm, long sCn, long sCb,
                             const float* bias, int bias_mode, int flags, int splitk, void* stream) {
    return jvae_gemm_launch(M, N, K, batch, A, sAm, sAk, sAb, B, sBk, sBn, sBb, C, sCm, sCn, sCb,
                            bias, bias_mode, flags, splitk, (hipStream_t)stream);
}
```

joint-vae_amd/csrc/jvae_internal.h:

```cpp
#pragma once
#include <hip/hip_runtime.h>

int jvae_gemm_launch(int M, int N, int K, int batch,
                     const float* A, long sAm, long sAk, long sAb,
                     const float* B, long sBk, long sBn, long sBb,
                     float* C, long sCm, long sCn, long sCb,
                     const float* bias, int bias_mode, int flags, int splitk, hipStream_t st);

int jvae_gemm_launch_ex(int M, int N, int K, int batch,
                        const float* A, long sAm, long sAk, long sAb,
                        const float* B, long sBk, long sBn, long sBb,
                        float* C, long sCm, long sCn, long sCb,
                        const float* bias, int bias_mode, int bias_div, int flags, int splitk, hipStream_t st);

int jvae_splitk_fold_qn(const float* part, const float* bias, float* y, int S, int N, int Cs, int Ps, hipStream_t st);
int jvae_splitk_fold(const float* part, const float* bias, float* y, int S, long MN, int N, int relu, int accumulate,
                     hipStream_t st, int bias_div = 1);

int jvae_gemm_launch_part(int M, int N, int K, int batch,
                          const float* A, long sAm, long sAk, long sAb,
                          const float* B, long sBk, long sBn, long sBb,
                          float* part, long sCm, long sCn, long sCb, long sCsplit, int want_splits, int* splits,
                          hipStream_t st);

struct InAff { const float* sc; const float* sh; int relu; };

struct ConvGeom {
    int N;
    int Cb, Hb, Wb;
    int Cs, Hs, Ws;
    int KH, KW, S, P;
};

int jvae_wgrad_slab_reduce(const float* slab, float* dw, int G, int Ca, int Cb, int accumulate, int swapflip, hipStream_t st,
                           int tapmajor = 0, int taps = 25);
```

joint-vae_amd/jvae_hip/lib.py:

```python
import ctypes
import os
from ctypes import c_char_p, c_float, c_int, c_long, c_longlong, c_size_t, c_void_p, POINTER

import torch

_HERE = os.path.dirname(os.path.abspath(__file__))
LIB_PATH = os.environ.get('JVAE_HIP_LIB') or os.path.join(_HERE, 'libjvae_hip.so')

_lib = None

P = c_void_p
_SIGS = {
    'jvae_version': (c_char_p, []),
    'jvae_gemm_f32': (c_int, [c_int] * 4 + [P, c_long, c_long, c_long] * 3 + [P, c_int, c_int, c_int, P]),
    'jvae_splitk_fold_f32': (c_int, [P, P, P, c_int, c_long, c_int, c_int, c_int, P]),
    'jvae_conv2d_workspace_bytes': (c_size_t, [c_int] * 11),
    'jvae_conv2d_set_split_bf16': (c_int, [c_int]),
    'jvae_conv2d_set_split_shape16': (c_int, [c_int]),
    'jvae_conv2d_out_shape': (c_int, [c_int] * 8 + [POINTER(c_int), POINTER(c_int)]),
    'jvae_conv2d_route': (c_int, [c_int] * 17 + [POINTER(c_int), POINTER(c_int), POINTER(c_size_t), POINTER(c_int), POINTER(c_int)]),
    'jvae_conv2d_kernel_name': (c_char_p, [c_int]),
    'jvae_conv2d_fwd_f32': (c_int, [P, P, P, P] + [c_int] * 11 + [P, c_size_t, P]),
    'jvae_conv2d_stats_splits': (c_int, [c_int] * 11),
    'jvae_conv2d_fwd_stats_f32': (c_int, [P, P, P, P, P, POINTER(c_int)] + [c_int] * 11 + [P, c_size_t, P]),
    'jvae_conv2d_dgrad_f32': (c_int, [P, P, P] + [c_int] * 11 + [P, c_size_t, P]),
    'jvae_conv2d_wgrad_f32': (c_int, [P, P, P, P, c_int] + [c_int] * 11 + [P, c_size_t, P]),
    'jvae_b8_pack_f32': (c_int, [P, P, c_int, c_int, c_long, P]),
    'jvae_b8_unpack_f32': (c_int, [P, P, c_int, c_int, c_long, c_int, P]),
    'jvae_conv2d_native_b8': (c_int, [c_int] * 11),
    'jvae_conv2d_workspace_bytes_b8': (c_size_t, [c_int] * 11),
    'jvae_conv2d_stats_splits_b8': (c_int, [c_int] * 11),
    'jvae_conv2d_fwd_b8': (c_int, [P, P, P, P, c_int, P, POINTER(c_int)] + [c_int] * 11 + [P, c_size_t, P]),
    'jvae_conv2d_dgrad_b8': (c_int, [P, P, P] + [c_int] * 11 + [P, c_size_t, P]),
    'jvae_conv2d_wgrad_b8': (c_int, [P, P, P, P, c_int] + [c_int] * 11 + [P, c_size_t, P]),
    'jvae_bn_workspace_bytes_b8': (c_size_t, [c_int]),
    'jvae_bn_plan_b8': (c_int, [c_int, c_int, c_long, POINTER(c_int), POINTER(c_int)]),
    'jvae_bn_fwd_b8': (c_int, [P] * 9 + [c_int, c_int, c_long, c_float, c_float, c_int, c_int, P, c_int, P, P, c_size_t, P]),
    'jvae_bn_bwd_b8': (c_int, [P] * 9 + [c_int, c_int, c_int, c_long, c_int, P, c_size_t, P]),
    'jvae_bn_finalize_b8': (c_int, [P] * 9 + [c_int, c_int, c_long, c_float, c_float, c_int, P, c_int, P, P, c_size_t, P]),
    'jvae_bn_sums_b8': (c_int, [P, P, P, c_int, c_int, c_long, P, c_size_t, P]),
    'jvae_bn_fwd_sync_b8': (c_int, [P] * 9 + [c_int, c_int, c_long, c_float, c_float, c_int, P, P, c_int, P, c_size_t, P]),
    'jvae_bn_bwd_sums_b8': (c_int, [P] * 7 + [c_int, c_int, c_long, c_int, P, c_size_t, P]),
    'jvae_bn_bwd_sync_b8': (c_int, [P] * 8 + [c_int, P, P, P, c_int, c_int, c_int, c_long, c_int, P, c_size_t, P]),
    'jvae_conv2d_affine_ok_b8': (c_int, [c_int] * 11),
    'jvae_conv2d_fwd_aff_b8': (c_int, [P, P, P, P, c_int, P, POINTER(c_int), P, P, c_int] + [c_int] * 11 + [P, c_size_t, P]),
    'jvae_conv2d_wgrad_aff_b8': (c_int, [P, P, P, P, c_int, P, P, c_int] + [c_int] * 11 + [P, c_size_t, P]),
    'jvae_relu_fwd_b8': (c_int, [P, P, c_long, P]),
    'jvae_relu_bwd_b8': (c_int, [P, P, P, c_long, P]),
    'jvae_bn_finalize_f32': (c_int, [P] * 10 + [c_int, c_int, c_int, c_float, c_float, c_int, P, c_int, P, P, c_size_t, P]),
    'jvae_conv2d_affine_ok': (c_int, [c_int] * 11),
    'jvae_conv2d_fwd_aff_f32': (c_int, [P, P, P, P, P, POINTER(c_int), P, P, c_int] + [c_int] * 11 + [P, c_size_t, P]),
    'jvae_conv2d_wgrad_aff_f32': (c_int, [P, P, P, P, c_int, P, P, c_int] + [c_int] * 11 + [P, c_size_t, P]),
    'jvae_pack_cache_configure': (c_int, [P, c_size_t]),
    'jvae_pack_cache_begin': (c_int, [P, c_longlong, P, c_int]),
    'jvae_pack_cache_end': (c_int, []),
    'jvae_pack_cache_pin': (c_int, []),
    'jvae_pack_cache_reset': (c_int, []),
    'jvae_pack_cache_stats': (c_int, [POINTER(c_int), POINTER(c_longlong), POINTER(c_longlong), POINTER(c_longlong)]),
    'jvae_channel_sum_workspace_bytes': (c_size_t, [c_int]),
    'jvae_channel_sum_f32': (c_int, [P, P, c_int, c_int, c_int, c_int, P, c_size_t, P]),
    'jvae_bn_workspace_bytes': (c_size_t, [c_int]),
    'jvae_bn_plan': (c_int, [c_int, c_int, c_int, POINTER(c_int), POINTER(c_int)]),
    'jvae_image_range': (c_int, [c_int, c_int, c_int, POINTER(c_int), POINTER(c_int)]),
    'jvae_bn_fwd_f32': (c_int, [P] * 9 + [c_int, c_int, c_int, c_float, c_float, c_int, c_int, P, c_size_t, P]),
    'jvae_bn_fwd_ext_f32': (c_int, [P] * 9 + [c_int, c_int, c_int, c_float, c_float, c_int, c_int, P, c_int, P, P, c_size_t, P]),
    'jvae_bn_sums_f32': (c_int, [P, P, P, c_int, c_int, c_int, P, c_size_t, P]),
    'jvae_bn_fwd_sync_f32': (c_int, [P] * 9 + [c_int, c_int, c_int, c_float, c_float, c_int, P, P, c_int, P, c_size_t, P]),
    'jvae_bn_bwd_sums_f32': (c_int, [P] * 7 + [c_int, c_int, c_int, c_int, P, c_size_t, P]),
    'jvae_bn_bwd_sync_f32': (c_int, [P] * 8 + [c_int, P, P, P, c_int, c_int, c_int, c_int, c_int, P]),
    'jvae_bn_bwd_f32': (c_int, [P] * 9 + [c_int, c_int, c_int, c_int, c_int, P, c_size_t, P]),
    'jvae_bn_eval_bwd_f32': (c_int, [P] * 7 + [c_int, c_int, c_int, c_float, c_int, P]),
    'jvae_act_fwd_f32': (c_int, [P, P, c_long, c_int, P]),
    'jvae_act_bwd_f32': (c_int, [P, P, P, c_long, c_int, P]),
    'jvae_dict_stats_f32': (c_int, [P, P, c_int, c_int, P]),
    'jvae_latent_fwd_f32': (c_int, [P] * 13 + [c_int] * 6 + [c_float] * 3 + [c_int, c_int, c_float, P]),
    'jvae_latent_bwd_f32': (c_int, [P] * 17 + [c_int] * 6 + [c_float] * 3 + [c_int, c_int, P, c_size_t, P]),
    'jvae_latent_fwd_wdev_f32': (c_int, [P] * 13 + [c_int] * 6 + [c_float] * 3 + [c_int, c_int, c_float, P, P]),
    'jvae_latent_bwd_wdev_f32': (c_int, [P] * 17 + [c_int] * 6 + [c_float] * 3 + [c_int, c_int, P, P, c_size_t, P]),
    'jvae_recon_fwd_f32': (c_int, [P, P, P, c_int, P, c_int, c_int, c_int, P]),
    'jvae_recon_bwd_f32': (c_int, [P, P, P, c_int, P, P, P, P, P, c_int, c_int, c_int, c_int, P, c_size_t, P]),
    'jvae_mse_rows_fwd_f32': (c_int, [P, P, P, c_int, c_int, c_int, P]),
    'jvae_mse_rows_bwd_f32': (c_int, [P, P, P, P, c_int, c_int, c_int, P]),
    'jvae_elbo_fwd_f32': (c_int, [P, P, P, P, c_int, P, P, P, P, c_int, c_int, c_int, c_float, c_float, P]),
    'jvae_elbo_bwd_f32': (c_int, [P, P, P, P, c_int, P, P, P, P, c_int, c_int, c_int, c_int, c_float, c_float, P, c_size_t, P]),
    'jvae_elbo_fwd_wdev_f32': (c_int, [P, P, P, P, c_int, P, P, P, P, c_int, c_int, c_int, c_float, c_float, P, P]),
    'jvae_elbo_bwd_wdev_f32': (c_int, [P, P, P, P, c_int, P, P, P, P, c_int, c_int, c_int, c_int, c_float, c_float, P, P, c_size_t, P]),
    'jvae_measures_dev_f32': (c_int, [P, c_long, P, P, P, c_int, c_int, P, c_int, P, c_int, c_int, P, P, P, P]),
    'jvae_loss_sums_f32': (c_int, [P, P, c_int, P, P]),
    'jvae_measures_f32': (c_int, [P, c_long, P, P, P, c_int, c_int, P, c_int, P, c_int, c_int, P, P, c_int, P, P]),
    'jvae_dropout_f32': (c_int, [P, P, c_long, c_float, c_long, P]),
    'jvae_dropout_dev_f32': (c_int, [P, P, c_long, c_float, P, c_long, P]),
    'jvae_iws_f32': (c_int, [P, P, P, P, P, c_int, c_int, c_int, c_int, c_int, c_int, P, P, P]),
    'jvae_xent_fwd_f32': (c_int, [P, P, P, c_int, c_int, c_int, P]),
    'jvae_xent_bwd_f32': (c_int, [P, P, P, P, c_int, c_int, c_int, P]),
    'jvae_augment_u8_f32': (c_int, [P, P, P, P, P, c_int, c_int, c_int, c_int, c_int, c_int, P]),
    'jvae_sqnorm_workspace_bytes': (c_size_t, []),
    'jvae_sqnorm_accum_f32': (c_int, [P, c_long, P, c_int, P, c_size_t, P]),
    'jvae_clip_scale_f32': (c_int, [P, c_long, P, c_float, P]),
    'jvae_adam_step_dev_f32': (c_int, [P, P, P, P, c_long, P, c_int, c_float, c_float, c_float, P, P, P]),
    'jvae_adam_step_f32': (c_int, [P, P, P, P, c_long] + [c_float] * 5 + [c_long, c_float, P, P, P]),
    'jvae_sgd_step_f32': (c_int, [P, P, P, c_long, c_float, c_float, c_int, c_float, c_int, c_float, P, P, P]),
    'jvae_pool2d_out_shape': (c_int, [c_int] * 5 + [POINTER(c_int), POINTER(c_int)]),
    'jvae_pool2d_fwd_f32': (c_int, [P, P, P, c_long] + [c_int] * 6 + [P]),
    'jvae_pool2d_bwd_f32': (c_int, [P, P, P, c_long] + [c_int] * 6 + [P]),
    'jvae_upsample_nearest_fwd_f32': (c_int, [P, P, c_long, c_int, c_int, c_int, P]),
    'jvae_upsample_nearest_bwd_f32': (c_int, [P, P, c_long, c_int, c_int, c_int, P]),
    'jvae_pool2d_fwd_b8': (c_int, [P, P, P, c_long] + [c_int] * 6 + [P]),
    'jvae_pool2d_bwd_b8': (c_int, [P, P, P, c_long] + [c_int] * 6 + [P]),
    'jvae_upsample_nearest_fwd_b8': (c_int, [P, P, c_long, c_int, c_int, c_int, P]),
    'jvae_upsample_nearest_bwd_b8': (c_int, [P, P, c_long, c_int, c_int, c_int, P]),
    'jvae_roc_workspace_bytes': (c_size_t, [c_int, c_long, c_long]),
    'jvae_roc_curve_f32': (c_int, [P] * 10 + [c_int, c_long, c_long, c_int, P, c_size_t, P]),
    'jvae_misclass_scores_f32': (c_int, [P] * 5 + [c_int, c_int, c_long, c_long, P]),
    'jvae_misclass_split_workspace_bytes': (c_size_t, [c_long]),
    'jvae_misclass_split_f32': (c_int, [P, P, P, P, c_int, c_long, P, c_size_t, P]),
    'jvae_misclass_confusion_f32': (c_int, [P] * 5 + [c_int, c_long, c_int, P]),
    'jvae_odin_head_f32': (c_int, [P, P, P, P, c_int, c_int, c_int, c_int, c_long, c_long, P]),
    'jvae_odin_perturb_f32': (c_int, [P, P, P, P, P, c_long, c_int, P]),
}


class JvaeHipError(RuntimeError):
    pass


def load():
    global _lib
    if _lib is not None:
        return _lib
    if not os.path.exists(LIB_PATH):
        raise JvaeHipError(f'{LIB_PATH} is missing: build it with `python -c "import __graft_entry__ as g; g.build()"` '
                           'or `make -C joint-vae_amd/csrc` (there is no CPU/PyTorch fallback)')
    lib = ctypes.CDLL(LIB_PATH)
    for name, (res, args) in _SIGS.items():
        fn = getattr(lib, name)
        fn.restype = res
        fn.argtypes = args
    _lib = lib
    return lib


def exported_symbols():
    return list(_SIGS)


_ERR = {-1: 'invalid argument', -2: 'unsupported configuration', -3: 'workspace too small'}


def check(rc, what):
    if rc != 0:
        msg = _ERR.get(rc, f'hipError_t {rc}')
        raise JvaeHipError(f'{what} failed: {msg}')


_raw_stream = getattr(torch._C, '_cuda_getCurrentRawStream', None)


def stream_ptr(device_index=None):
    if _raw_stream is not None:
        return _raw_stream(torch.cuda.current_device() if device_index is None else device_index)
    return torch.cuda.current_stream().cuda_stream


def ptr(t):
    if t is None:
        return None
    if not t.is_cuda:
        raise JvaeHipError('jvae_hip ops need tensors resident on the GPU (no CPU fallback); got device '
                           + str(t.device))
    if not t.is_contiguous():
        raise JvaeHipError('jvae_hip ops need contiguous tensors')
    return t.data_ptr()


_workspaces = {}
_side_streams = {}


def side_stream(device):
    idx = device.index if device.index is not None else torch.cuda.current_device()
    st = _side_streams.get(idx)
    if st is None:
        _side_streams[idx] = st = torch.cuda.Stream(device=idx)
    return st


def join_side_stream(device=None):
    for idx, st in _side_streams.items():
        if device is None or device.index in (None, idx):
            torch.cuda.current_stream(idx).wait_stream(st)


def workspace(nbytes, device):
    idx = device.index if device.index is not None else torch.cuda.current_device()
    key = (idx, stream_ptr(idx))
    ws = _workspaces.get(key)
    if ws is None or ws.numel() < nbytes:
        _workspaces[key] = ws = torch.empty(max(int(nbytes), 1 << 20), dtype=torch.uint8, device=device)
    return ws


PACK_CACHE_BYTES = int(os.environ.get('JVAE_PACK_CACHE_MB', '64')) << 20
_pack_cache = {}
span_depth = 0
span_hold = 0


def pack_cache_begin(weights, device):
    if not PACK_CACHE_BYTES:
        return
    lib = load()
    idx = device.index if device.index is not None else torch.cuda.current_device()
    if idx not in _pack_cache:
        if _pack_cache:
            check(lib.jvae_pack_cache_configure(None, 0), 'jvae_pack_cache_configure')
            _pack_cache[idx] = None
        else:
            buf = torch.empty(PACK_CACHE_BYTES + 256, dtype=torch.uint8, device=device)
            off = (-buf.data_ptr()) % 256
            _pack_cache[idx] = buf
            check(lib.jvae_pack_cache_configure(buf.data_ptr() + off, PACK_CACHE_BYTES), 'jvae_pack_cache_configure')
    if _pack_cache[idx] is None:
        return
    addrs = tuple(w.data_ptr() for w in weights)
    arr = (ctypes.c_void_p * max(len(addrs), 1))(*addrs)
    check(lib.jvae_pack_cache_begin(stream_ptr(idx), hash(addrs), arr, len(addrs)), 'jvae_pack_cache_begin')


def pack_cache_end():
    if _lib is not None and _pack_cache:
        _lib.jvae_pack_cache_end()


def pack_cache_pin():
    if _lib is not None and _pack_cache and PACK_CACHE_BYTES:
        _lib.jvae_pack_cache_pin()


def pack_cache_stats():
    lib = load()
    e, h, m, r = c_int(), c_longlong(), c_longlong(), c_longlong()
    lib.jvae_pack_cache_stats(ctypes.byref(e), ctypes.byref(h), ctypes.byref(m), ctypes.byref(r))
    return {'entries': e.value, 'hits': h.value, 'misses': m.value, 'refreshes': r.value}
```

joint-vae_amd/jvae_hip/ops.py:

```python
import collections
import contextlib
import ctypes
import math
from ctypes import byref, c_int, c_size_t

import torch

from . import lib as L

RELU, SIGMOID, IDENT, LEAKY = 1, 2, 0, 3
BN_ACT = {IDENT: 0, RELU: 1, LEAKY: 2}
OVERLAP_WGRAD = True
ACT_KIND = {'relu': RELU, 'sigmoid': SIGMOID, 'linear': IDENT, 'leaky': LEAKY, None: IDENT}


def _c(t):
    return t if t.is_contiguous() else t.contiguous()


def _f32(t, what):
    if t.dtype != torch.float32:
        raise L.JvaeHipError(f'{what}: fp32 expected, got {t.dtype}')
    return t


def _grad_slot(param):
    if param is None or not isinstance(param, torch.nn.Parameter):
        return None
    g = param.grad
    if g is None or not g.is_contiguous() or g.dtype != torch.float32 or g.shape != param.shape or not g.is_cuda:
        return None
    return g


def _join_after_backward():
    torch.autograd.Variable._execution_engine.queue_callback(L.join_side_stream)


def _close_span_after_backward():
    if not L.span_hold:
        torch.autograd.Variable._execution_engine.queue_callback(L.pack_cache_end)


def gemm(M, N, K, A, sA, B, sB, C, sC, bias=None, bias_mode=0, flags=0, splitk=1, batch=1):
    lib = L.load()
    rc = lib.jvae_gemm_f32(M, N, K, batch, L.ptr(A), *sA, L.ptr(B), *sB, L.ptr(C), *sC,
                           L.ptr(bias), bias_mode, flags, splitk, L.stream_ptr())
    L.check(rc, 'jvae_gemm_f32')


def channel_sum(t, N, C, P, out=None, accumulate=False):
    lib = L.load()
    if out is None:
        out = torch.empty(C, device=t.device, dtype=torch.float32)
    ws = L.workspace(lib.jvae_channel_sum_workspace_bytes(C), t.device)
    L.check(lib.jvae_channel_sum_f32(L.ptr(t), L.ptr(out), N, C, P, int(accumulate), L.ptr(ws), ws.numel(), L.stream_ptr()),
            'channel_sum')
    return out


def _linear_split(R, O, I):
    tiles = ((R + 63) // 64) * ((O + 63) // 64)
    if tiles >= 128 or I < 512:
        return 1
    for S in (32, 16, 8, 4, 2):
        if tiles * S <= 1024 and I % S == 0 and I // S >= 128:
            return S
    return 1


class _Linear(torch.autograd.Function):

    @staticmethod
    def forward(ctx, x, w, b, act):
        x2 = _c(_f32(x, 'linear').reshape(-1, x.shape[-1]))
        w_in = w
        w = _c(w)
        R, I = x2.shape
        O = w.shape[0]
        y = torch.empty((R, O), device=x.device, dtype=torch.float32)
        S = _linear_split(R, O, I)
        if S > 1:
            part = torch.empty((S, R, O), device=x.device, dtype=torch.float32)
            Ks = I // S
            gemm(R, O, Ks, x2, (I, 1, Ks), w, (1, I, Ks), part, (O, 1, R * O), batch=S)
            L.check(L.load().jvae_splitk_fold_f32(L.ptr(part), L.ptr(b), L.ptr(y), S, R * O, O, int(act == RELU), 0,
                                                  L.stream_ptr()), 'jvae_splitk_fold_f32')
        else:
            gemm(R, O, I, x2, (I, 1, 0), w, (1, I, 0), y, (O, 1, 0), bias=b, bias_mode=1 if b is not None else 0,
                 flags=2 if act == RELU else 0)
        if act in (SIGMOID, LEAKY):
            L.check(L.load().jvae_act_fwd_f32(L.ptr(y), L.ptr(y), y.numel(), act, L.stream_ptr()), 'act_fwd')
        ctx.save_for_backward(x2, w, y if act != IDENT else None)
        ctx.act = act
        ctx.has_bias = b is not None
        ctx.xshape = x.shape
        ctx.w_ref, ctx.b_ref = w_in, b
        return y.reshape(*x.shape[:-1], O)

    @staticmethod
    def backward(ctx, gy):
        x2, w, y = ctx.saved_tensors
        lib = L.load()
        R, I = x2.shape
        O = w.shape[0]
        gy = _c(gy.reshape(R, O))
        if ctx.act != IDENT:
            g = torch.empty_like(gy)
            L.check(lib.jvae_act_bwd_f32(L.ptr(gy), L.ptr(y), L.ptr(g), gy.numel(), ctx.act, L.stream_ptr()), 'act_bwd')
            gy = g
        gx = gw = gb = None
        if ctx.needs_input_grad[0]:
            gx = torch.empty((R, I), device=gy.device, dtype=torch.float32)
            gemm(R, I, O, gy, (O, 1, 0), w, (I, 1, 0), gx, (I, 1, 0))
            gx = gx.reshape(ctx.xshape)
        if ctx.needs_input_grad[1]:
            slot = _grad_slot(ctx.w_ref)
            gw = slot if slot is not None else torch.zeros((O, I), device=gy.device, dtype=torch.float32)
            S = _linear_split(O, I, R)
            if S > 1:
                part = torch.empty((S, O, I), device=gy.device, dtype=torch.float32)
                Rs = R // S
                gemm(O, I, Rs, gy, (1, O, Rs * O), x2, (I, 1, Rs * I), part, (I, 1, O * I), batch=S)
                L.check(lib.jvae_splitk_fold_f32(L.ptr(part), None, L.ptr(gw), S, O * I, I, 0, 1, L.stream_ptr()),
                        'jvae_splitk_fold_f32')
            else:
                gemm(O, I, R, gy, (1, O, 0), x2, (I, 1, 0), gw, (I, 1, 0), flags=1)
            if slot is not None:
                gw = None
        if ctx.has_bias and ctx.needs_input_grad[2]:
            slot = _grad_slot(ctx.b_ref)
            if slot is not None:
                channel_sum(gy, R, O, 1, out=slot, accumulate=True)
            else:
                gb = channel_sum(gy, R, O, 1)
        return gx, gw, gb, None


def linear(x, w, b=None, act=IDENT):
    return _Linear.apply(x, w, b, act)


_GEOM_CACHE = {}


def _geom_query(name, geom):
    key = (name, geom)
    r = _GEOM_CACHE.get(key)
    if r is None:
        _GEOM_CACHE[key] = r = getattr(L.load(), name)(*geom)
    return r


class ConvSpec:
    __slots__ = ('cin', 'cout', 'k', 's', 'p', 'op', 'transposed')

    def __init__(self, cin, cout, k, s, p, op=0, transposed=False):
        self.cin, self.cout, self.k, self.s, self.p, self.op, self.transposed = cin, cout, k, s, p, op, bool(transposed)

    def out_hw(self, H, W):
        key = ('hw', self.k, self.s, self.p, self.op, self.transposed, H, W)
        r = _GEOM_CACHE.get(key)
        if r is None:
            oh, ow = c_int(), c_int()
            rc = L.load().jvae_conv2d_out_shape(H, W, self.k, self.k, self.s, self.p, self.op, int(self.transposed),
                                                byref(oh), byref(ow))
            L.check(rc, 'jvae_conv2d_out_shape')
            _GEOM_CACHE[key] = r = (oh.value, ow.value)
        return r

    def geom(self, N, H, W):
        return (N, self.cin, H, W, self.cout, self.k, self.k, self.s, self.p, self.op, int(self.transposed))


def _conv_ws(geom, device):
    nbytes = _geom_query('jvae_conv2d_workspace_bytes', geom)
    ws = L.workspace(nbytes, device)
    return ws, ws.numel()


def conv_fwd_raw(x, w, b, spec):
    N, _, H, W = x.shape
    oh, ow = spec.out_hw(H, W)
    y = torch.empty((N, spec.cout, oh, ow), device=x.device, dtype=torch.float32)
    geom = spec.geom(N, H, W)
    ws, nb = _conv_ws(geom, x.device)
    rc = L.load().jvae_conv2d_fwd_f32(L.ptr(x), L.ptr(w), L.ptr(b), L.ptr(y), *geom, L.ptr(ws), nb, L.stream_ptr())
    L.check(rc, 'jvae_conv2d_fwd_f32')
    return y


def conv_fwd_stats_raw(x, w, b, spec):
    lib = L.load()
    N, _, H, W = x.shape
    geom = spec.geom(N, H, W)
    cap = _geom_query('jvae_conv2d_stats_splits', geom)
    if cap <= 0:
        return conv_fwd_raw(x, w, b, spec), None, 0
    oh, ow = spec.out_hw(H, W)
    y = torch.empty((N, spec.cout, oh, ow), device=x.device, dtype=torch.float32)
    stats = torch.empty((spec.cout * cap * 2,), device=x.device, dtype=torch.float32)
    ws, nb = _conv_ws(geom, x.device)
    ns = c_int(0)
    rc = lib.jvae_conv2d_fwd_stats_f32(L.ptr(x), L.ptr(w), L.ptr(b), L.ptr(y), L.ptr(stats), byref(ns), *geom,
                                       L.ptr(ws), nb, L.stream_ptr())
    L.check(rc, 'jvae_conv2d_fwd_stats_f32')
    return y, (stats if ns.value > 0 else None), ns.value


def conv_affine_ok(spec, N, H, W):
    return bool(_geom_query('jvae_conv2d_affine_ok', spec.geom(N, H, W)))


ConvRoute = collections.namedtuple('ConvRoute', 'kernel swap ws splits aff_ok')
ROUTE_DIR = {'fwd': 1, 'dgrad': 2, 'wgrad': 4}
ROUTE_LAYOUT = {'f32': 0, 'b8': 1}


def conv_route(spec, N, H, W, direction, layout='f32', bias=False, stats=False, y_f32=False, aff=0):
    lib = L.load()
    k, sw, ns, ok, ws = c_int(), c_int(), c_int(), c_int(), c_size_t()
    rc = lib.jvae_conv2d_route(ROUTE_DIR[direction], ROUTE_LAYOUT[layout], int(bias), int(stats), int(y_f32), int(aff),
                               *spec.geom(N, H, W), byref(k), byref(sw), byref(ws), byref(ns), byref(ok))
    L.check(rc, 'jvae_conv2d_route')
    return ConvRoute(lib.jvae_conv2d_kernel_name(k.value).decode(), bool(sw.value), ws.value, ns.value, bool(ok.value))


class LaunchProbe:

    def __init__(self, match):
        self.match, self.events, self.armed = match, [], False

    def times_ms(self):
        return [a.elapsed_time(b) for a, b in self.events]


FWD_AFF_PROBE = None


def conv_fwd_aff_raw(x, w, b, spec, aff, want_stats):
    lib = L.load()
    N, _, H, W = x.shape
    geom = spec.geom(N, H, W)
    oh, ow = spec.out_hw(H, W)
    y = torch.empty((N, spec.cout, oh, ow), device=x.device, dtype=torch.float32)
    stats, ns = None, c_int(0)
    if want_stats:
        cap = _geom_query('jvae_conv2d_stats_splits', geom)
        if cap > 0:
            stats = torch.empty((spec.cout * cap * 2,), device=x.device, dtype=torch.float32)
    ws, nb = _conv_ws(geom, x.device)
    probe = FWD_AFF_PROBE
    timed = probe is not None and probe.armed and probe.match(spec, N, H)
    if timed:
        ev = (torch.cuda.Event(enable_timing=True), torch.cuda.Event(enable_timing=True))
        ev[0].record()
    rc = lib.jvae_conv2d_fwd_aff_f32(L.ptr(x), L.ptr(w), L.ptr(b), L.ptr(y), L.ptr(stats), byref(ns),
                                     L.ptr(aff[0]), L.ptr(aff[1]), int(aff[2]), *geom, L.ptr(ws), nb, L.stream_ptr())
    if timed:
        ev[1].record()
        probe.events.append(ev)
    L.check(rc, 'jvae_conv2d_fwd_aff_f32')
    return y, (stats if ns.value > 0 else None), ns.value


def conv_dgrad_raw(gy, w, spec, xshape):
    N, _, H, W = xshape
    gx = torch.empty(xshape, device=gy.device, dtype=torch.float32)
    geom = spec.geom(N, H, W)
    ws, nb = _conv_ws(geom, gy.device)
    rc = L.load().jvae_conv2d_dgrad_f32(L.ptr(gy), L.ptr(w), L.ptr(gx), *geom, L.ptr(ws), nb, L.stream_ptr())
    L.check(rc, 'jvae_conv2d_dgrad_f32')
    return gx


def conv_wgrad_raw(x, gy, spec, wshape, want_bias, w_slot=None, b_slot=None, aff=None):
    N, _, H, W = x.shape
    inplace = w_slot is not None and (b_slot is not None or not want_bias)
    gw = w_slot if inplace else torch.empty(wshape, device=x.device, dtype=torch.float32)
    gb = None
    if want_bias:
        gb = b_slot if inplace else torch.empty(spec.cout, device=x.device, dtype=torch.float32)
    geom = spec.geom(N, H, W)
    ws, nb = _conv_ws(geom, x.device)
    if aff is not None:
        rc = L.load().jvae_conv2d_wgrad_aff_f32(L.ptr(x), L.ptr(gy), L.ptr(gw), L.ptr(gb), int(inplace),
                                                L.ptr(aff[0]), L.ptr(aff[1]), int(aff[2]), *geom, L.ptr(ws), nb,
                                                L.stream_ptr())
    else:
        rc = L.load().jvae_conv2d_wgrad_f32(L.ptr(x), L.ptr(gy), L.ptr(gw), L.ptr(gb), int(inplace), *geom, L.ptr(ws), nb,
                                            L.stream_ptr())
    L.check(rc, 'jvae_conv2d_wgrad_f32')
    return (None, None) if inplace else (gw, gb)


FWD, DGRAD, WGRAD = 1, 2, 4


class Layout:
    sfx = '_f32'
    ws_sfx = ''
    acts = BN_ACT

    def dims(self, x, C):
        N, C = x.shape[0], x.shape[1]
        return N, C, x.numel() // max(N * C, 1)

    def coef_width(self, C):
        return C

    def prep(self, x, what):
        return _c(_f32(x, what))

    def to_f32(self, t, C):
        return t

    def from_f32(self, t):
        return t

    def native(self, spec, N, H, W):
        return FWD | DGRAD | WGRAD

    def affine_ok(self, spec, N, H, W):
        return conv_affine_ok(spec, N, H, W)

    def conv_fwd(self, x, w, b, spec, want_stats, aff, out_f32):
        if aff is not None:
            return conv_fwd_aff_raw(x, w, b, spec, aff, want_stats)
        if want_stats:
            return conv_fwd_stats_raw(x, w, b, spec)
        return conv_fwd_raw(x, w, b, spec), None, 0

    def conv_dgrad(self, gy, w, spec, N, H, W):
        return conv_dgrad_raw(gy, w, spec, (N, spec.cin, H, W))

    def conv_wgrad(self, *args):
        return conv_wgrad_raw(*args)

    def bn(self, name, *args, ws=None):
        name += self.sfx
        extra = () if ws is None else (L.ptr(ws), ws.numel())
        L.check(getattr(L.load(), name)(*args, *extra, L.stream_ptr()), name)

    def bn_workspace(self, C, device):
        return L.workspace(getattr(L.load(), 'jvae_bn_workspace_bytes' + self.ws_sfx)(C), device)

    def bn_fwd(self, *args, ext, ws):
        if ext[0] is None:
            self.bn('jvae_bn_fwd', *args, ws=ws)
        else:
            self.bn('jvae_bn_fwd_ext', *args, *ext, ws=ws)

    def coef_args(self, coef):
        return L.ptr(coef[0]), L.ptr(coef[1])

    def bn_bwd_sync(self, *args, ws):
        self.bn('jvae_bn_bwd_sync', *args)


F32 = Layout()


def layout_of(t):
    return _b8.B8 if _b8.is_b8(t) else F32


class _Conv(torch.autograd.Function):

    @staticmethod
    def forward(ctx, x, w, b, spec, dead_bias, stats_out, aff, out_f32):
        lay = layout_of(x)
        x = lay.prep(x, 'conv')
        if not L.span_depth:
            L.pack_cache_end()
        ctx.w_ref, ctx.b_ref = w, b
        w = _c(w)
        native = lay.native(spec, x.shape[0], x.shape[2], x.shape[3])
        if aff is not None and (native & (FWD | WGRAD)) != FWD | WGRAD:
            raise L.JvaeHipError('a deferred BatchNorm needs native forward and weight-gradient kernels (conv_affine_ok)')
        want_stats = stats_out is not None
        if native & FWD:
            y, st, ns = lay.conv_fwd(x, w, b, spec, want_stats, aff, out_f32)
        else:
            y, st, ns = F32.conv_fwd(lay.to_f32(x, spec.cin), w, b, spec, want_stats, None, False)
            y = y if out_f32 else lay.from_f32(y)
        if want_stats:
            stats_out['stats'], stats_out['nsplit'], stats_out['pivot'] = st, ns, b
        ctx.save_for_backward(x, w)
        ctx.lay, ctx.native, ctx.spec, ctx.out_f32, ctx.aff = lay, native, spec, out_f32, aff
        ctx.has_bias = b is not None
        ctx.dead_bias = dead_bias
        return y

    @staticmethod
    def backward(ctx, gy):
        x, w = ctx.saved_tensors
        lay, spec = ctx.lay, ctx.spec
        N, H, W = x.shape[0], x.shape[2], x.shape[3]
        gys = {F32 if ctx.out_f32 else lay: _c(gy)}

        def gy_in(want):
            if want not in gys:
                have, g = next(iter(gys.items()))
                gys[want] = want.from_f32(g) if have is F32 else have.to_f32(g, spec.cout)
            return gys[want]
        gx = gw = gb = None
        _close_span_after_backward()
        want_b = ctx.has_bias and ctx.needs_input_grad[2] and not ctx.dead_bias
        wgrad = ctx.needs_input_grad[1] or want_b
        on_side = False
        if wgrad:
            w_slot = _grad_slot(ctx.w_ref)
            b_slot = _grad_slot(ctx.b_ref) if want_b else None
            on_side = (OVERLAP_WGRAD and ctx.needs_input_grad[0] and w_slot is not None
                       and (b_slot is not None or not want_b))
        if ctx.needs_input_grad[0]:
            dl = lay if ctx.native & DGRAD else F32
            gyd = gy_in(dl)
        if on_side:
            side = L.side_stream(x.device)
            side.wait_stream(torch.cuda.current_stream(x.device))
        if ctx.needs_input_grad[0]:
            gx = dl.conv_dgrad(gyd, w, spec, N, H, W)
            gx = gx if dl is lay else lay.from_f32(gx)
        if wgrad:
            with torch.cuda.stream(side) if on_side else contextlib.nullcontext():
                wl = lay if ctx.native & WGRAD else F32
                xw = x if wl is lay else lay.to_f32(x, spec.cin)
                gw, gb = wl.conv_wgrad(xw, gy_in(wl), spec, w.shape, want_b, w_slot, b_slot, ctx.aff)
            if on_side:
                for t in (x, xw, *gys.values(), *(ctx.aff[:2] if ctx.aff is not None else ())):
                    t.record_stream(side)
                _join_after_backward()
        if ctx.dead_bias and ctx.has_bias and ctx.needs_input_grad[2] and _grad_slot(ctx.b_ref) is None:
            gb = torch.zeros_like(ctx.b_ref)
        return gx, gw, gb, None, None, None, None, None


def conv2d(x, w, b, spec, dead_bias=False, stats_out=None, aff=None, out_f32=False):
    return _Conv.apply(x, w, b, spec, dead_bias, stats_out, aff, out_f32)


def _ext_args(ext, training):
    if ext is None or ext.get('stats') is None or not training:
        return None, 0, None
    return L.ptr(ext['stats']), int(ext['nsplit']), L.ptr(ext.get('pivot'))


def _bn_save(ctx, lay, training, relu, dims, x, gamma, beta, mean, invstd, rm, rv, eps):
    ctx.lay = lay
    ctx.relu, ctx.dims = relu, dims
    ctx.eval_eps = None if training else float(eps)
    if training:
        ctx.save_for_backward(x, gamma, beta, mean, invstd)
        ctx.g_ref, ctx.b_ref = gamma, beta
    else:
        ctx.save_for_backward(x, gamma, beta, rm, rv)


def _bn_eval_backward(ctx, gy):
    if ctx.lay is not F32:
        raise NotImplementedError('backward through an eval-mode BatchNorm is built for the fp32 layout only')
    x, gamma, beta, rm, rv = ctx.saved_tensors
    N, C, P = ctx.dims
    gy = _c(gy)
    gx = torch.empty_like(x)
    L.check(L.load().jvae_bn_eval_bwd_f32(L.ptr(gy), L.ptr(x), L.ptr(gamma), L.ptr(beta), L.ptr(rm), L.ptr(rv), L.ptr(gx),
                                          N, C, P, ctx.eval_eps, int(ctx.relu), L.stream_ptr()), 'jvae_bn_eval_bwd_f32')
    return gx, None, None, None, None, None, None, None, None, None, None, None


def _bn_param_grads(ctx, C, device):
    sg, sb = _grad_slot(ctx.g_ref), _grad_slot(ctx.b_ref)
    if sg is not None and sb is not None:
        return sg, sb, True
    return torch.empty(C, device=device, dtype=torch.float32), torch.empty(C, device=device, dtype=torch.float32), False


class _BatchNormAct(torch.autograd.Function):

    @staticmethod
    def forward(ctx, x, gamma, beta, rm, rv, nbt, training, relu, momentum, eps, ext, C):
        lay = layout_of(x)
        x = lay.prep(x, 'batchnorm')
        N, C, P = lay.dims(x, C)
        y = torch.empty_like(x)
        mean = torch.empty(C, device=x.device, dtype=torch.float32)
        invstd = torch.empty(C, device=x.device, dtype=torch.float32)
        lay.bn_fwd(L.ptr(x), L.ptr(gamma), L.ptr(beta), L.ptr(rm), L.ptr(rv), L.ptr(nbt), L.ptr(y), L.ptr(mean), L.ptr(invstd),
                   N, C, P, momentum, eps, int(training), int(relu), ext=_ext_args(ext, training),
                   ws=lay.bn_workspace(C, x.device))
        _bn_save(ctx, lay, training, relu, (N, C, P), x, gamma, beta, mean, invstd, rm, rv, eps)
        return y

    @staticmethod
    def backward(ctx, gy):
        if ctx.eval_eps is not None:
            return _bn_eval_backward(ctx, gy)
        x, gamma, beta, mean, invstd = ctx.saved_tensors
        N, C, P = ctx.dims
        gy = _c(gy)
        gx = torch.empty_like(x)
        gg, gb, inplace = _bn_param_grads(ctx, C, x.device)
        ctx.lay.bn('jvae_bn_bwd', L.ptr(gy), L.ptr(x), L.ptr(gamma), L.ptr(beta), L.ptr(mean), L.ptr(invstd), L.ptr(gx),
                   L.ptr(gg), L.ptr(gb), int(inplace), N, C, P, int(ctx.relu), ws=ctx.lay.bn_workspace(C, x.device))
        if inplace:
            gg = gb = None
        return gx, gg, gb, None, None, None, None, None, None, None, None, None


def batchnorm_act(x, gamma, beta, running_mean, running_var, num_batches_tracked, training, relu,
                  momentum=0.1, eps=1e-5, ext=None, C=None):
    return _BatchNormAct.apply(x, gamma, beta, running_mean, running_var, num_batches_tracked, training, relu,
                               momentum, eps, ext, C)


class _BatchNormDefer(torch.autograd.Function):

    @staticmethod
    def forward(ctx, x, gamma, beta, rm, rv, nbt, training, relu, momentum, eps, ext, C):
        lay = layout_of(x)
        x = lay.prep(x, 'batchnorm')
        N, C, P = lay.dims(x, C)
        mean = torch.empty(C, device=x.device, dtype=torch.float32)
        invstd = torch.empty(C, device=x.device, dtype=torch.float32)
        coef = torch.empty((2, lay.coef_width(C)), device=x.device, dtype=torch.float32)
        lay.bn('jvae_bn_finalize', L.ptr(x), L.ptr(gamma), L.ptr(beta), L.ptr(rm), L.ptr(rv), L.ptr(nbt), L.ptr(mean),
               L.ptr(invstd), *lay.coef_args(coef), N, C, P, momentum, eps, int(training), *_ext_args(ext, training),
               ws=lay.bn_workspace(C, x.device))
        _bn_save(ctx, lay, training, relu, (N, C, P), x, gamma, beta, mean, invstd, rm, rv, eps)
        ctx.mark_non_differentiable(coef)
        ctx.set_materialize_grads(False)
        return x.view_as(x), coef

    @staticmethod
    def backward(ctx, gy, _gcoef):
        return _BatchNormAct.backward(ctx, gy)


def batchnorm_defer(x, gamma, beta, running_mean, running_var, num_batches_tracked, training, relu,
                    momentum=0.1, eps=1e-5, ext=None, C=None):
    xa, coef = _BatchNormDefer.apply(x, gamma, beta, running_mean, running_var, num_batches_tracked, training, relu,
                                     momentum, eps, ext, C)
    return xa, (coef[0], coef[1], relu)


class _SyncBatchNormAct(torch.autograd.Function):

    @staticmethod
    def forward(ctx, x, gamma, beta, rm, rv, nbt, relu, momentum, eps, world, group, C):
        import torch.distributed as dist
        lay = layout_of(x)
        x = lay.prep(x, 'sync batchnorm')
        N, C, P = lay.dims(x, C)
        ws = lay.bn_workspace(C, x.device)
        pivot = rm.detach().clone()
        sums = torch.empty((C, 2), device=x.device, dtype=torch.float32)
        lay.bn('jvae_bn_sums', L.ptr(x), L.ptr(pivot), L.ptr(sums), N, C, P, ws=ws)
        dist.all_reduce(sums, op=dist.ReduceOp.SUM, group=group)
        y = torch.empty_like(x)
        mean = torch.empty(C, device=x.device, dtype=torch.float32)
        invstd = torch.empty(C, device=x.device, dtype=torch.float32)
        lay.bn('jvae_bn_fwd_sync', L.ptr(x), L.ptr(gamma), L.ptr(beta), L.ptr(rm), L.ptr(rv), L.ptr(nbt), L.ptr(y),
               L.ptr(mean), L.ptr(invstd), N, C, P, momentum, eps, int(relu), L.ptr(sums), L.ptr(pivot), int(world), ws=ws)
        ctx.save_for_backward(x, gamma, beta, mean, invstd)
        ctx.lay, ctx.cfg = lay, (N, C, P, relu, int(world), group)
        ctx.g_ref, ctx.b_ref = gamma, beta
        return y

    @staticmethod
    def backward(ctx, gy):
        import torch.distributed as dist
        x, gamma, beta, mean, invstd = ctx.saved_tensors
        N, C, P, relu, world, group = ctx.cfg
        lay = ctx.lay
        gy = _c(gy)
        ws = lay.bn_workspace(C, x.device)
        local = torch.empty((C, 2), device=x.device, dtype=torch.float32)
        lay.bn('jvae_bn_bwd_sums', L.ptr(gy), L.ptr(x), L.ptr(gamma), L.ptr(beta), L.ptr(mean), L.ptr(invstd), L.ptr(local),
               N, C, P, int(relu), ws=ws)
        glob = local.clone()
        dist.all_reduce(glob, op=dist.ReduceOp.SUM, group=group)
        gx = torch.empty_like(x)
        gg, gb, inplace = _bn_param_grads(ctx, C, x.device)
        lay.bn_bwd_sync(L.ptr(gy), L.ptr(x), L.ptr(gamma), L.ptr(beta), L.ptr(mean), L.ptr(invstd), L.ptr(local),
                        L.ptr(glob), world, L.ptr(gx), L.ptr(gg), L.ptr(gb), int(inplace), N, C, P, int(relu), ws=ws)
        if inplace:
            gg = gb = None
        return gx, gg, gb, None, None, None, None, None, None, None, None, None


def sync_batchnorm_act(x, gamma, beta, running_mean, running_var, num_batches_tracked, relu, momentum, eps, world, group=None,
                       C=None):
    return _SyncBatchNormAct.apply(x, gamma, beta, running_mean, running_var, num_batches_tracked, relu, momentum, eps,
                                   world, group, C)


class _Act(torch.autograd.Function):
    @staticmethod
    def forward(ctx, x, kind):
        x = _c(_f32(x, 'act'))
        y = torch.empty_like(x)
        L.check(L.load().jvae_act_fwd_f32(L.ptr(x), L.ptr(y), x.numel(), kind, L.stream_ptr()), 'act_fwd')
        ctx.save_for_backward(y)
        ctx.kind = kind
        return y

    @staticmethod
    def backward(ctx, gy):
        y, = ctx.saved_tensors
        gy = _c(gy)
        gx = torch.empty_like(gy)
        L.check(L.load().jvae_act_bwd_f32(L.ptr(gy), L.ptr(y), L.ptr(gx), gy.numel(), ctx.kind, L.stream_ptr()), 'act_bwd')
        return gx, None


def act(x, kind):
    if kind == IDENT:
        if not x.is_cuda:
            raise L.JvaeHipError('jvae_hip ops need tensors resident on the GPU (no CPU fallback)')
        return x
    return _Act.apply(x, kind)


class _Dropout(torch.autograd.Function):

    @staticmethod
# ... 628 lines not shown
```

Baseline: 144,900.

## Add implicit-im2col GEMM for generic conv path with fused input BN affine

The generic conv forward and weight-grad paths can now feed the GEMM directly from the input tensor through an implicit-im2col descriptor instead of first writing an unfold buffer. The input batch-norm affine and activation is also folded into the unfold or implicit load, so generic-routed convs are now accepted for affine fusion and skip the separate BN-apply pass. This is meant to cut memory traffic from materialising the column buffer and normalised activations. The cost is index arithmetic with magic-number division inside the GEMM loads, plus extra routing conditions and fallbacks.

```diff
diff --git a/include/jvae_hip.h b/include/jvae_hip.h
--- a/include/jvae_hip.h
+++ b/include/jvae_hip.h
@@ -22,6 +22,7 @@
                                    int transposed);
 int jvae_conv2d_set_split_bf16(int mode);
 int jvae_conv2d_set_split_shape16(int on);
+int jvae_conv2d_set_generic_implicit(int on);
 int jvae_conv2d_out_shape(int H, int W, int KH, int KW, int S, int P, int OP, int transposed, int* OH, int* OW);
 int jvae_conv2d_route(int dir, int layout, int bias, int stats, int y_f32, int aff_kind,
                       int N, int Cin, int H, int W, int Cout, int KH, int KW, int S, int P, int OP, int transposed,
@@ -81,6 +82,7 @@
                          const float* ext_stats, int ext_nsplit, const float* ext_pivot,
                          void* ws, size_t ws_bytes, void* stream);
 int jvae_conv2d_affine_ok(int N, int Cin, int H, int W, int Cout, int KH, int KW, int S, int P, int OP, int transposed);
+int jvae_conv2d_generic_affine_ok(int N, int Cin, int H, int W, int Cout, int KH, int KW, int S, int P, int OP, int transposed);
 int jvae_conv2d_fwd_aff_f32(const float* x, const float* w, const float* bias, float* y, float* stats, int* nsplit,
                             const float* in_scale, const float* in_shift, int in_relu,
                             int N, int Cin, int H, int W, int Cout, int KH, int KW, int S, int P, int OP, int transposed,
diff --git a/joint-vae_amd/csrc/conv_api.hip b/joint-vae_amd/csrc/conv_api.hip
--- a/joint-vae_amd/csrc/conv_api.hip
+++ b/joint-vae_amd/csrc/conv_api.hip
@@ -11,6 +11,9 @@
 bool affine_ok(const ConvGeom& g, int transposed, ConvDir other, const ConvRoute& r) {
     return r.aff_ok && route(g, transposed, other, {false, false, false, 1}).aff_ok;
 }
+bool affine_accepted(const ConvGeom& g, int transposed, ConvDir other, const ConvRoute& r) {
+    return affine_ok(g, transposed, other, r) || (r.k == CK_GENERIC && jvae_conv_generic_aff(g, transposed));
+}
 
 int fwd_f32(const float* x, const float* w, const float* bias, float* y, float* stats, int* nsplit, const InAff* aff,
             int N, int Cin, int H, int W, int Cout, int KH, int KW, int S, int P, int OP, int transposed,
@@ -19,7 +22,7 @@
     if (nsplit) *nsplit = 0;
     if (!jvae_make_geom(N, Cin, H, W, Cout, KH, KW, S, P, OP, transposed, &g, &oh, &ow)) return JVAE_EINVAL;
     const ConvRoute r = route(g, transposed, CONV_FWD, {bias != nullptr, stats != nullptr, false, jvae_aff_kind(aff)});
-    if (aff && !affine_ok(g, transposed, CONV_WGRAD, r)) return JVAE_ENOTSUP;
+    if (aff && !affine_accepted(g, transposed, CONV_WGRAD, r)) return JVAE_ENOTSUP;
     if (N == 0) return 0;
     if (jvae_ws_short(r, ws, ws_bytes)) return JVAE_EWORKSPACE;
     return jvae_conv_run_fwd(r, g, x, w, bias, y, (float*)ws, ws_bytes, (hipStream_t)stream, stats, nsplit, aff);
@@ -32,7 +35,7 @@
     if (!dw || (N > 0 && (!x || !dy))) return JVAE_EINVAL;
     if (!jvae_make_geom(N, Cin, H, W, Cout, KH, KW, S, P, OP, transposed, &g, &oh, &ow)) return JVAE_EINVAL;
     const ConvRoute r = route(g, transposed, CONV_WGRAD, {false, false, false, jvae_aff_kind(aff)});
-    if (aff && !affine_ok(g, transposed, CONV_FWD, r)) return JVAE_ENOTSUP;
+    if (aff && !affine_accepted(g, transposed, CONV_FWD, r)) return JVAE_ENOTSUP;
     if (N > 0 && jvae_ws_short(r, ws, ws_bytes)) return JVAE_EWORKSPACE;
     hipStream_t st = (hipStream_t)stream;
     if (!accumulate) {
@@ -58,6 +61,7 @@
 
 int jvae_conv2d_set_split_bf16(int mode) { return jvae_conv5_x3_set(mode); }
 int jvae_conv2d_set_split_shape16(int on) { return jvae_conv5_x3_set_shape16(on); }
+int jvae_conv2d_set_generic_implicit(int on) { return jvae_conv_generic_implicit_set(on); }
 
 size_t jvae_conv2d_workspace_bytes(int N, int Cin, int H, int W, int Cout, int KH, int KW, int S, int P, int OP,
                                    int transposed) {
@@ -128,6 +132,12 @@
     return affine_ok(g, transposed, CONV_WGRAD, route(g, transposed, CONV_FWD, {false, false, false, 1})) ? 1 : 0;
 }
 
+int jvae_conv2d_generic_affine_ok(int N, int Cin, int H, int W, int Cout, int KH, int KW, int S, int P, int OP, int transposed) {
+    ConvGeom g; int oh, ow;
+    if (!jvae_make_geom(N, Cin, H, W, Cout, KH, KW, S, P, OP, transposed, &g, &oh, &ow)) return 0;
+    return jvae_conv_generic_aff(g, transposed) && jvae_fold_fwd_implicit(g) ? 1 : 0;
+}
+
 int jvae_conv2d_fwd_aff_f32(const float* x, const float* w, const float* bias, float* y, float* stats, int* nsplit,
                             const float* in_scale, const float* in_shift, int in_relu,
                             int N, int Cin, int H, int W, int Cout, int KH, int KW, int S, int P, int OP, int transposed,
diff --git a/joint-vae_amd/csrc/conv_dispatch.h b/joint-vae_amd/csrc/conv_dispatch.h
--- a/joint-vae_amd/csrc/conv_dispatch.h
+++ b/joint-vae_amd/csrc/conv_dispatch.h
@@ -4,11 +4,13 @@
 
 size_t jvae_conv_generic_ws(const ConvGeom& g);
 int jvae_fold_fwd(const ConvGeom& g, const float* xb, const float* w, const float* bias, float* ys,
-                  float* ws, size_t ws_bytes, hipStream_t st);
+                  float* ws, size_t ws_bytes, hipStream_t st, const InAff* aff = nullptr);
 int jvae_fold_bwd(const ConvGeom& g, const float* ys, const float* w, const float* bias, float* xb,
                   float* ws, size_t ws_bytes, hipStream_t st);
 int jvae_fold_wgrad(const ConvGeom& g, const float* xb, const float* ys, float* dw,
-                    float* ws, size_t ws_bytes, hipStream_t st);
+                    float* ws, size_t ws_bytes, hipStream_t st, const InAff* aff = nullptr);
+int jvae_conv_generic_implicit_set(int on);
+bool jvae_fold_fwd_implicit(const ConvGeom& g);
 size_t jvae_channel_sum_ws_bytes(int C);
 int jvae_channel_sum(const float* t, float* out, int N, int C, int P, int accumulate, float* ws, size_t ws_bytes,
                      hipStream_t st);
@@ -98,6 +100,7 @@
     *aff_q = p_is_x ? nullptr : aff;
 }
 
+bool jvae_conv_generic_aff(const ConvGeom& g, int transposed);
 size_t jvae_conv_ws(const ConvGeom& g, int transposed);
 int jvae_conv_run_fwd(const ConvRoute& r, const ConvGeom& g, const float* in, const float* w, const float* bias, float* out,
                       float* ws, size_t ws_bytes, hipStream_t st, float* stats = nullptr, int* nsplit = nullptr,
diff --git a/joint-vae_amd/csrc/conv_dispatch.hip b/joint-vae_amd/csrc/conv_dispatch.hip
--- a/joint-vae_amd/csrc/conv_dispatch.hip
+++ b/joint-vae_amd/csrc/conv_dispatch.hip
@@ -134,6 +134,12 @@
     return fwd_route(g, transposed, dir, layout == CONV_B8, f);
 }
 
+bool jvae_conv_generic_aff(const ConvGeom& g, int transposed) {
+    if (transposed) return false;
+    const CallFlags f{false, false, false, 1};
+    return fwd_route(g, 0, CONV_FWD, false, f).k == CK_GENERIC && wgrad_route(g, 0, false, f).k == CK_GENERIC;
+}
+
 size_t jvae_conv_ws(const ConvGeom& g, int transposed) {
     size_t a = max_sz(jvae_conv_generic_ws(g), jvae_channel_sum_ws_bytes(g.Cb > g.Cs ? g.Cb : g.Cs));
     for (ConvDir d : {CONV_FWD, CONV_DGRAD, CONV_WGRAD}) a = max_sz(a, jvae_conv_route(g, transposed, d, CONV_F32, {}).ws);
@@ -172,7 +178,9 @@
             return jvae_splitk_fold(ws, nullptr, out, S, outf, g.Cs, 0, 0, st);
         }
         case CK_GENERIC:
-            return r.swap ? jvae_fold_bwd(g, in, w, bias, out, ws, ws_bytes, st) : jvae_fold_fwd(g, in, w, bias, out, ws, ws_bytes, st);
+            if (aff && r.swap) return JVAE_ENOTSUP;
+            return r.swap ? jvae_fold_bwd(g, in, w, bias, out, ws, ws_bytes, st)
+                          : jvae_fold_fwd(g, in, w, bias, out, ws, ws_bytes, st, aff);
         default: return JVAE_ENOTSUP;
     }
 }
@@ -201,7 +209,9 @@
             if (rc) return rc;
             return jvae_splitk_fold(ws, nullptr, dw, S, outf, cols, 0, 1, st);
         }
-        case CK_GENERIC: return jvae_fold_wgrad(g, big, small, dw, ws, ws_bytes, st);
+        case CK_GENERIC:
+            if (aff && transposed) return JVAE_ENOTSUP;
+            return jvae_fold_wgrad(g, big, small, dw, ws, ws_bytes, st, aff);
         default: return JVAE_ENOTSUP;
     }
 }
diff --git a/joint-vae_amd/csrc/conv_generic.hip b/joint-vae_amd/csrc/conv_generic.hip
--- a/joint-vae_amd/csrc/conv_generic.hip
+++ b/joint-vae_amd/csrc/conv_generic.hip
@@ -1,11 +1,12 @@
 #include "common.h"
 #include "jvae_internal.h"
+#include "conv_dispatch.h"
 
 namespace {
 
 __global__ __launch_bounds__(256) void unfold_kernel(const float* __restrict__ xb, float* __restrict__ col,
                                                      ConvGeom g, int n0, int nimg, long sn, long sk, long sq,
-                                                     int kfast) {
+                                                     int kfast, InAff aff) {
     const int Kd = g.Cb * g.KH * g.KW, Ps = g.Hs * g.Ws;
     const long total = (long)nimg * Kd * Ps;
     for (long i = (long)blockIdx.x * blockDim.x + threadIdx.x; i < total; i += (long)gridDim.x * blockDim.x) {
@@ -16,15 +17,17 @@
         const int hs = q / g.Ws, ws = q % g.Ws;
         const int hb = hs * g.S + kh - g.P, wb = ws * g.S + kw - g.P;
         float v = 0.f;
-        if (hb >= 0 && hb < g.Hb && wb >= 0 && wb < g.Wb)
+        if (hb >= 0 && hb < g.Hb && wb >= 0 && wb < g.Wb) {
             v = xb[(((long)(n0 + n) * g.Cb + cb) * g.Hb + hb) * g.Wb + wb];
+            if (aff.sc) v = jvae_act(fmaf(v, aff.sc[cb], aff.sh[cb]), jvae_act_kind(aff.relu));
+        }
         col[(long)n * sn + (long)k * sk + (long)q * sq] = v;
     }
 }
 
 template <bool KFAST>
 __global__ __launch_bounds__(256) void unfold4_kernel(const float* __restrict__ xb, float* __restrict__ col,
-                                                      ConvGeom g, int n0, int nimg) {
+                                                      ConvGeom g, int n0, int nimg, InAff aff) {
     const unsigned Kd = g.Cb * g.KH * g.KW, Ps = g.Hs * g.Ws, KK = g.KH * g.KW;
     const unsigned inner4 = (KFAST ? Kd : Ps) / 4;
     const unsigned total = (KFAST ? Ps * (unsigned)nimg : (unsigned)nimg * Kd) * inner4;
@@ -43,6 +46,8 @@
             const int hb = (int)(hs * g.S + kh) - g.P;
             const int wb = (int)((KFAST ? ws : ws + e) * g.S + kw) - g.P;
             v[e] = (hb >= 0 && hb < g.Hb && wb >= 0 && wb < g.Wb) ? src[((long)cb * g.Hb + hb) * g.Wb + wb] : 0.f;
+            if (aff.sc && hb >= 0 && hb < g.Hb && wb >= 0 && wb < g.Wb)
+                v[e] = jvae_act(fmaf(v[e], aff.sc[cb], aff.sh[cb]), jvae_act_kind(aff.relu));
             if (KFAST && ++kw == (unsigned)g.KW) { kw = 0; if (++kh == (unsigned)g.KH) { kh = 0; ++cb; } }
         }
         *reinterpret_cast<f32x4*>(col + (long)i * 4) = v;
@@ -145,17 +150,19 @@
     return (int)(b > 16384 ? 16384 : (b < 1 ? 1 : b));
 }
 
-int launch_unfold(const float* xb, float* col, const ConvGeom& g, int n0, int nimg, bool kfast, hipStream_t st) {
+int launch_unfold(const float* xb, float* col, const ConvGeom& g, int n0, int nimg, bool kfast, hipStream_t st,
+                  const InAff* aff_) {
+    const InAff aff = aff_ ? *aff_ : InAff{nullptr, nullptr, 0};
     const long Kd = (long)g.Cb * g.KH * g.KW, Ps = (long)g.Hs * g.Ws, total = (long)nimg * Kd * Ps;
     const bool vec = total < (1L << 31) && (kfast ? Kd % 4 == 0 : g.Ws % 4 == 0) && ((uintptr_t)col & 15) == 0;
     if (vec && kfast)
-        hipLaunchKernelGGL(unfold4_kernel<true>, dim3(grid_for4(total / 4)), dim3(256), 0, st, xb, col, g, n0, nimg);
+        hipLaunchKernelGGL(unfold4_kernel<true>, dim3(grid_for4(total / 4)), dim3(256), 0, st, xb, col, g, n0, nimg, aff);
     else if (vec)
-        hipLaunchKernelGGL(unfold4_kernel<false>, dim3(grid_for4(total / 4)), dim3(256), 0, st, xb, col, g, n0, nimg);
+        hipLaunchKernelGGL(unfold4_kernel<false>, dim3(grid_for4(total / 4)), dim3(256), 0, st, xb, col, g, n0, nimg, aff);
     else if (kfast)
-        hipLaunchKernelGGL(unfold_kernel, dim3(grid_for(total)), dim3(256), 0, st, xb, col, g, n0, nimg, Kd, 1L, (long)nimg * Kd, 1);
+        hipLaunchKernelGGL(unfold_kernel, dim3(grid_for(total)), dim3(256), 0, st, xb, col, g, n0, nimg, Kd, 1L, (long)nimg * Kd, 1, aff);
     else
-        hipLaunchKernelGGL(unfold_kernel, dim3(grid_for(total)), dim3(256), 0, st, xb, col, g, n0, nimg, Kd * Ps, Ps, 1L, 0);
+        hipLaunchKernelGGL(unfold_kernel, dim3(grid_for(total)), dim3(256), 0, st, xb, col, g, n0, nimg, Kd * Ps, Ps, 1L, 0, aff);
     JVAE_LAUNCH_CHECK();
     return 0;
 }
@@ -195,6 +202,20 @@
 
 inline long wgrad_part_floats(const ConvGeom& g) { return (long)g.Cs * g.Cb * g.KH * g.KW; }
 
+int g_implicit = 1;
+
+}
+
+int jvae_conv_generic_implicit_set(int on) {
+    const int old = g_implicit;
+    g_implicit = on ? 1 : 0;
+    return old;
+}
+
+bool jvae_fold_fwd_implicit(const ConvGeom& g) {
+    GemmImp im;
+    return g_implicit && jvae_conv5_x3_enabled() && pixel_batched(g) && (long)g.Cb * g.KH * g.KW >= 64 &&
+           jvae_gemm_imp_make(g, nullptr, nullptr, &im);
 }
 
 size_t jvae_conv_generic_ws(const ConvGeom& g) {
@@ -219,12 +240,31 @@
 }
 
 int jvae_fold_fwd(const ConvGeom& g, const float* xb, const float* w, const float* bias, float* ys,
-                  float* ws, size_t ws_bytes, hipStream_t st) {
+                  float* ws, size_t ws_bytes, hipStream_t st, const InAff* aff) {
     const int Kd = g.Cb * g.KH * g.KW, Ps = g.Hs * g.Ws;
     if (pixel_batched(g)) {
         if (ws_bytes < (size_t)col_floats_per_image(g) * 4 * g.N) return JVAE_EWORKSPACE;
-        { const int rc = launch_unfold(xb, ws, g, 0, g.N, true, st); if (rc) return rc; }
+        GemmImp im;
+        const GemmImp* imp = jvae_fold_fwd_implicit(g) && jvae_gemm_imp_make(g, xb, aff, &im) ? &im : nullptr;
         const int want = fwd_slices(g);
+        if (imp) {
+            int rc;
+            if (want > 1) {
+                const long colf = (long)col_floats_per_image(g) * g.N, outf = (long)g.N * g.Cs * Ps;
+                if (ws_bytes < 4 * (size_t)(colf + want * outf)) return JVAE_EWORKSPACE;
+                float* part = ws + colf;
+                int S = 0;
+                rc = jvae_gemm_launch_part(g.N, g.Cs, Kd, Ps, xb, Kd, 1, (long)g.N * Kd, w, 1, Kd, 0,
+                                           part, g.Cs, 1, (long)g.N * g.Cs, outf, want, &S, st, imp, 1);
+                if (!rc) return jvae_splitk_fold_qn(part, bias, ys, S, g.N, g.Cs, Ps, st);
+            } else {
+                rc = jvae_gemm_launch(g.N, g.Cs, Kd, Ps, xb, Kd, 1, (long)g.N * Kd, w, 1, Kd, 0,
+                                      ys, (long)g.Cs * Ps, Ps, 1, bias, bias ? 1 : 0, 0, 1, st, imp, 1);
+                if (!rc) return 0;
+            }
+            if (rc != JVAE_ENOTSUP) return rc;
+        }
+        { const int rc = launch_unfold(xb, ws, g, 0, g.N, true, st, aff); if (rc) return rc; }
         if (want > 1) {
             const long colf = (long)col_floats_per_image(g) * g.N, outf = (long)g.N * g.Cs * Ps;
             if (ws_bytes < 4 * (size_t)(colf + want * outf)) return JVAE_EWORKSPACE;
@@ -242,7 +282,7 @@
     if (chunk < 1) return JVAE_EWORKSPACE;
     for (int n0 = 0; n0 < g.N; n0 += chunk) {
         const int ni = (g.N - n0 < chunk) ? g.N - n0 : chunk;
-        { const int rc = launch_unfold(xb, ws, g, n0, ni, false, st); if (rc) return rc; }
+        { const int rc = launch_unfold(xb, ws, g, n0, ni, false, st, aff); if (rc) return rc; }
         int rc = jvae_gemm_launch(g.Cs, Ps, Kd, ni, w, Kd, 1, 0, ws, Ps, 1, (long)Kd * Ps,
                                   ys + (long)n0 * g.Cs * Ps, Ps, 1, (long)g.Cs * Ps, bias, bias ? 2 : 0, 0, 1, st);
         if (rc) return rc;
@@ -296,11 +336,11 @@
 }
 
 int jvae_fold_wgrad(const ConvGeom& g, const float* xb, const float* ys, float* dw,
-                    float* ws, size_t ws_bytes, hipStream_t st) {
+                    float* ws, size_t ws_bytes, hipStream_t st, const InAff* aff) {
     const int Kd = g.Cb * g.KH * g.KW, Ps = g.Hs * g.Ws;
     if (pixel_batched(g)) {
         if (ws_bytes < (size_t)col_floats_per_image(g) * 4 * g.N) return JVAE_EWORKSPACE;
-        { const int rc = launch_unfold(xb, ws, g, 0, g.N, true, st); if (rc) return rc; }
+        if (!wgrad_joint(g)) { const int rc = launch_unfold(xb, ws, g, 0, g.N, true, st, aff); if (rc) return rc; }
         if (wgrad_joint(g)) {
             const int S = wgrad_slices(g);
             const long colf = (long)col_floats_per_image(g) * g.N, ytf = (long)g.N * g.Cs * Ps;
@@ -310,8 +350,17 @@
             hipLaunchKernelGGL(small_transpose_kernel, dim3(grid_for(ytf)), dim3(256), 0, st, ys, yt, g.N, g.Cs, Ps);
             JVAE_LAUNCH_CHECK();
             const long Ks = (long)Ps * g.N / S;
-            int rc = jvae_gemm_launch(g.Cs, Kd, (int)Ks, S, yt, 1, g.Cs, Ks * g.Cs, ws, Kd, 1, Ks * Kd,
+            GemmImp im;
+            int rc = JVAE_ENOTSUP;
+            if (g_implicit && jvae_gemm_imp_make(g, xb, aff, &im))
+                rc = jvae_gemm_launch(g.Cs, Kd, (int)Ks, S, yt, 1, g.Cs, Ks * g.Cs, xb, Kd, 1, Ks * Kd,
+                                      part, Kd, 1, (long)g.Cs * Kd, nullptr, 0, 0, 1, st, &im, 2);
+            if (rc == JVAE_ENOTSUP) {
+                rc = launch_unfold(xb, ws, g, 0, g.N, true, st, aff);
+                if (rc) return rc;
+                rc = jvae_gemm_launch(g.Cs, Kd, (int)Ks, S, yt, 1, g.Cs, Ks * g.Cs, ws, Kd, 1, Ks * Kd,
                                       part, Kd, 1, (long)g.Cs * Kd, nullptr, 0, 0, 1, st);
+            }
             if (rc) return rc;
             return jvae_splitk_fold(part, nullptr, dw, S, (long)g.Cs * Kd, Kd, 0, 1, st);
         }
@@ -332,7 +381,7 @@
     float* part = ws + chunk * colf;
     for (int n0 = 0; n0 < g.N; n0 += (int)chunk) {
         const int ni = (g.N - n0 < chunk) ? g.N - n0 : (int)chunk;
-        { const int rc = launch_unfold(xb, ws, g, n0, ni, false, st); if (rc) return rc; }
+        { const int rc = launch_unfold(xb, ws, g, n0, ni, false, st, aff); if (rc) return rc; }
         const float* a = ys + (long)n0 * g.Cs * Ps;
         if (ni == 1) {
             const int rc = jvae_gemm_launch(g.Cs, Kd, Ps, 1, a, Ps, 1, 0, ws, 1, Ps, 0, dw, Kd, 1, 0, nullptr, 0, 1, 1, st);
diff --git a/joint-vae_amd/csrc/gemm.hip b/joint-vae_amd/csrc/gemm.hip
--- a/joint-vae_amd/csrc/gemm.hip
+++ b/joint-vae_amd/csrc/gemm.hip
@@ -23,6 +23,8 @@
     long sCsplit;
     int vecA, vecB;
     int xcd;
+    int imp_side;
+    GemmImp imp;
 };
 
 template <bool VEC>
@@ -207,6 +209,44 @@
     }
 }
 
+__device__ __forceinline__ unsigned imp_div(unsigned a, int d, unsigned m) { return d == 1 ? a : __umulhi(a, m); }
+
+__device__ __forceinline__ f32x4 imp_load4(const GemmImp& im, unsigned R, unsigned k, bool ok, unsigned* meta) {
+    const unsigned q = imp_div(R, im.Nimg, im.mN), n = R - q * im.Nimg;
+    const unsigned hs = imp_div(q, im.Ws, im.mWs), ws = q - hs * im.Ws;
+    unsigned cb = imp_div(k, im.KK, im.mKK);
+    const unsigned t = k - cb * im.KK;
+    unsigned kh = imp_div(t, im.KW, im.mKW), kw = t - kh * im.KW;
+    const int h0 = (int)(hs * im.S) - im.P, w0 = (int)(ws * im.S) - im.P;
+    const unsigned base = n * (unsigned)(im.Cb * im.Hb * im.Wb);
+    unsigned m = cb << 8;
+    f32x4 v;
+#pragma unroll
+    for (int e = 0; e < 4; ++e) {
+        const int hb = h0 + (int)kh, wb = w0 + (int)kw;
+        const bool in = ok && (unsigned)hb < (unsigned)im.Hb && (unsigned)wb < (unsigned)im.Wb;
+        v[e] = im.x[in ? base + (cb * im.Hb + hb) * im.Wb + wb : 0u];
+        m |= (in ? 1u : 0u) << e;
+        if (++kw == (unsigned)im.KW) { kw = 0; if (++kh == (unsigned)im.KH) { kh = 0; ++cb; m |= (unsigned)(e + 1) << 4; } }
+    }
+    *meta = m;
+    return v;
+}
+
+__device__ __forceinline__ f32x4 imp_finish(const GemmImp& im, f32x4 v, unsigned meta, const float* tab) {
+    const unsigned c0 = meta >> 8, sw = (meta >> 4) & 7u;
+#pragma unroll
+    for (int e = 0; e < 4; ++e) {
+        float x = v[e];
+        if (im.sc) {
+            const unsigned c = c0 + ((sw && (unsigned)e >= sw) ? 1u : 0u);
+            x = jvae_act(fmaf(x, tab[c], tab[JVAE_GEMM_IMP_CH + c]), im.act);
+        }
+        v[e] = ((meta >> e) & 1u) ? x : 0.f;
+    }
+    return v;
+}
+
 template <bool KC>
 struct GxImg {
     static constexpr int PITCH = KC ? (BKX * 2 + 16) : (64 * 2 + 64);
@@ -214,8 +254,9 @@
     static constexpr int BYTES = PITCH * ROWS;
 };
 
-template <bool AK, bool BNC, int DEPTH = 1>
+template <bool AK, bool BNC, int DEPTH = 1, int IMP = 0>
 __global__ __launch_bounds__(256, 4) void gemm_x3_kernel(GemmP p) {
+    static_assert(IMP == 0 || (DEPTH > 1 && (IMP == 1 ? AK : BNC)), "the implicit operand is k-contiguous, deep form only");
     using IA = GxImg<AK>;
     using IB = GxImg<!BNC>;
     constexpr int BM = 64, BN = 64, G4 = BM * BKX / 4 / 256;
@@ -223,6 +264,7 @@
     extern __shared__ __attribute__((aligned(16))) unsigned char gx_lds[];
     unsigned char* As = gx_lds;
     unsigned char* Bs = gx_lds + 3 * IA::BYTES;
+    const float* imp_tab = reinterpret_cast<const float*>(gx_lds + 3 * (IA::BYTES + IB::BYTES));
 
     const int tid = threadIdx.x, lane = tid & 63, wave = tid >> 6;
     const int half = lane >> 5, l31 = lane & 31;
@@ -245,6 +287,13 @@
 #pragma unroll
     for (int r = 0; r < 16; ++r) acc[r] = 0.f;
     f32x4 ra[DEPTH][G4], rb[DEPTH][G4];
+    unsigned rmeta[IMP ? DEPTH : 1][G4];
+    if constexpr (IMP != 0) {
+        if (p.imp.sc) {
+            float* tab = reinterpret_cast<float*>(gx_lds + 3 * (IA::BYTES + IB::BYTES));
+            for (int c = threadIdx.x; c < p.imp.Cb; c += 256) { tab[c] = p.imp.sc[c]; tab[JVAE_GEMM_IMP_CH + c] = p.imp.sh[c]; }
+        }
+    }
 
     auto coordA = [&](int g, int k0, int* fast, int* slow) {
         if (AK) { *fast = k0 + (tid % KQX) * 4; *slow = m0 + tid / KQX + g * (256 / KQX); }
@@ -263,11 +312,19 @@
             if constexpr (DEPTH > 1) {
                 int f, sl;
                 coordA(g, k0, &f, &sl);
-                const float* sa = AK ? A + (long)sl * p.sAm + f : A + (long)sl * p.sAk + f;
-                ra[st][g] = *reinterpret_cast<const f32x4*>(okA(f, sl) ? sa : A);
+                if constexpr (IMP == 1) {
+                    ra[st][g] = imp_load4(p.imp, (unsigned)(batch * p.imp.rows + sl), (unsigned)f, okA(f, sl), &rmeta[st][g]);
+                } else {
+                    const float* sa = AK ? A + (long)sl * p.sAm + f : A + (long)sl * p.sAk + f;
+                    ra[st][g] = *reinterpret_cast<const f32x4*>(okA(f, sl) ? sa : A);
+                }
                 coordB(g, k0, &f, &sl);
-                const float* sb = BNC ? B + (long)sl * p.sBk + f : B + (long)sl * p.sBn + f;
-                rb[st][g] = *reinterpret_cast<const f32x4*>(okB(f, sl) ? sb : B);
+                if constexpr (IMP == 2) {
+                    rb[st][g] = imp_load4(p.imp, (unsigned)(batch * p.imp.rows + sl), (unsigned)f, okB(f, sl), &rmeta[st][g]);
+                } else {
+                    const float* sb = BNC ? B + (long)sl * p.sBk + f : B + (long)sl * p.sBn + f;
+                    rb[st][g] = *reinterpret_cast<const f32x4*>(okB(f, sl) ? sb : B);
+                }
                 continue;
             }
             if (AK) {
@@ -306,6 +363,8 @@
                 if (!okA(f, sl)) va = f32x4{0.f, 0.f, 0.f, 0.f};
                 coordB(g, k0, &f, &sl);
                 if (!okB(f, sl)) vb = f32x4{0.f, 0.f, 0.f, 0.f};
+                if constexpr (IMP == 1) va = imp_finish(p.imp, va, rmeta[st][g], imp_tab);
+                if constexpr (IMP == 2) vb = imp_finish(p.imp, vb, rmeta[st][g], imp_tab);
             }
             gx_u32x2 sa[3], sb[3];
             gx_split4(va, sa);
@@ -400,18 +459,18 @@
     }
 }
 
-template <bool AK, bool BNC, int DEPTH>
+template <bool AK, bool BNC, int DEPTH, int IMP = 0>
 int launch_x3_variant(const GemmP& p, int batch, hipStream_t st) {
-    constexpr int LDS = 3 * (GxImg<AK>::BYTES + GxImg<!BNC>::BYTES);
+    constexpr int LDS = 3 * (GxImg<AK>::BYTES + GxImg<!BNC>::BYTES) + (IMP ? 2 * JVAE_GEMM_IMP_CH * 4 : 0);
     static bool attr_set = false;
     if (!attr_set) {
-        hipError_t e = hipFuncSetAttribute(reinterpret_cast<const void*>(&gemm_x3_kernel<AK, BNC, DEPTH>),
+        hipError_t e = hipFuncSetAttribute(reinterpret_cast<const void*>(&gemm_x3_kernel<AK, BNC, DEPTH, IMP>),
                                            hipFuncAttributeMaxDynamicSharedMemorySize, LDS);
         if (e != hipSuccess) return (int)e;
         attr_set = true;
     }
     dim3 grid(cdiv(p.N, 64), cdiv(p.M, 64), batch * p.splitk), block(256);
-    hipLaunchKernelGGL((gemm_x3_kernel<AK, BNC, DEPTH>), grid, block, LDS, st, p);
+    hipLaunchKernelGGL((gemm_x3_kernel<AK, BNC, DEPTH, IMP>), grid, block, LDS, st, p);
     JVAE_LAUNCH_CHECK();
     return 0;
 }
@@ -420,6 +479,12 @@
 int launch_x3_ab(const GemmP& p, int batch, hipStream_t st) {
     const bool deep = p.vecA && p.vecB && p.K % 4 == 0
                       && (AK || p.M % 4 == 0) && (!BNC || p.N % 4 == 0);
+    if (p.imp_side) {
+        if (!deep) return JVAE_ENOTSUP;
+        if constexpr (AK && !BNC) { if (p.imp_side == 1) return launch_x3_variant<true, false, 3, 1>(p, batch, st); }
+        if constexpr (!AK && BNC) { if (p.imp_side == 2) return launch_x3_variant<false, true, 3, 2>(p, batch, st); }
+        return JVAE_ENOTSUP;
+    }
     if (deep) return launch_x3_variant<AK, BNC, 3>(p, batch, st);
     return launch_x3_variant<AK, BNC, 1>(p, batch, st);
 }
@@ -434,6 +499,20 @@
     return launch_x3_ab<false, false>(p, batch, st);
 }
 
+inline int set_imp(GemmP& p, const GemmImp* imp, int side, int K) {
+    p.imp_side = 0;
+    if (!imp || !side) return 0;
+    const long Kd = (long)imp->Cb * imp->KK;
+    const long sb = side == 1 ? p.sAb : p.sBb;
+    const bool dense = side == 1 ? (p.sAk == 1 && p.sAm == Kd) : (p.sBn == 1 && p.sBk == Kd);
+    if (!dense || sb % Kd != 0 || !(K >= 64 && jvae_conv5_x3_enabled())) return JVAE_ENOTSUP;
+    p.imp = *imp;
+    p.imp.rows = (int)(sb / Kd);
+    p.imp_side = side;
+    (side == 1 ? p.vecA : p.vecB) = 1;
+    return 0;
+}
+
 inline bool gemm_x3_on(int K) {
     return K >= 64 && jvae_conv5_x3_enabled();
 }
@@ -444,16 +523,18 @@
                      const float* A, long sAm, long sAk, long sAb,
                      const float* B, long sBk, long sBn, long sBb,
                      float* C, long sCm, long sCn, long sCb,
-                     const float* bias, int bias_mode, int flags, int splitk, hipStream_t st) {
+                     const float* bias, int bias_mode, int flags, int splitk, hipStream_t st,
+                     const GemmImp* imp, int imp_side) {
     return jvae_gemm_launch_ex(M, N, K, batch, A, sAm, sAk, sAb, B, sBk, sBn, sBb, C, sCm, sCn, sCb, bias, bias_mode, 1,
-                               flags, splitk, st);
+                               flags, splitk, st, imp, imp_side);
 }
 
 int jvae_gemm_launch_ex(int M, int N, int K, int batch,
                         const float* A, long sAm, long sAk, long sAb,
                         const float* B, long sBk, long sBn, long sBb,
                         float* C, long sCm, long sCn, long sCb,
-                        const float* bias, int bias_mode, int bias_div, int flags, int splitk, hipStream_t st) {
+                        const float* bias, int bias_mode, int bias_div, int flags, int splitk, hipStream_t st,
+                        const GemmImp* imp, int imp_side) {
     if (M <= 0 || N <= 0 || batch <= 0) return 0;
     if (K < 0 || !A || !B || !C) return JVAE_EINVAL;
     if (bias_mode && !bias) return JVAE_EINVAL;
@@ -478,17 +559,35 @@
     const bool ak = (sAk == 1), bnc = (sBn == 1);
     p.vecA = aligned16(A) && (sAb % 4 == 0) && (ak ? (sAm % 4 == 0) : (sAm == 1 && sAk % 4 == 0));
     p.vecB = aligned16(B) && (sBb % 4 == 0) && (bnc ? (sBk % 4 == 0) : (sBk == 1 && sBn % 4 == 0));
+    if (const int rc = set_imp(p, imp, imp_side, K)) return rc;
     if (gemm_x3_on(K)) return launch_x3(p, batch, st);
     const long tiles128 = (long)cdiv(M, 128) * cdiv(N, 128) * batch * splitk;
     if (M > 64 && N > 64 && tiles128 >= 512) return launch_tile<128, 128>(p, batch, st);
     return launch_tile<64, 64>(p, batch, st);
 }
 
+bool jvae_gemm_imp_make(const ConvGeom& g, const float* x, const InAff* aff, GemmImp* im) {
+    const long KK = (long)g.KH * g.KW, Kd = KK * g.Cb, Ps = (long)g.Hs * g.Ws;
+    const long lim = 1L << 32;
+    if (g.N < 1 || KK < 4 || Kd % 4 != 0 || g.Cb > JVAE_GEMM_IMP_CH) return false;
+    if ((long)g.N * g.Cb * g.Hb * g.Wb >= (1L << 31) || Kd * KK >= lim || Ps * g.N * g.N >= lim) return false;
+    auto magic = [](int d) { return (unsigned)(0xffffffffu / (unsigned)d + 1u); };
+    im->x = x;
+    im->sc = aff ? aff->sc : nullptr;
+    im->sh = aff ? aff->sh : nullptr;
+    im->act = aff ? jvae_act_kind(aff->relu) : JVAE_ACT_NONE;
+    im->Cb = g.Cb; im->Hb = g.Hb; im->Wb = g.Wb; im->KH = g.KH; im->KW = g.KW; im->KK = (int)KK;
+    im->Ws = g.Ws; im->S = g.S; im->P = g.P; im->Nimg = g.N;
+    im->rows = 0;
+    im->mKK = magic((int)KK); im->mKW = magic(g.KW); im->mN = magic(g.N); im->mWs = magic(g.Ws);
+    return true;
+}
+
 int jvae_gemm_launch_part(int M, int N, int K, int batch,
                           const float* A, long sAm, long sAk, long sAb,
                           const float* B, long sBk, long sBn, long sBb,
                           float* part, long sCm, long sCn, long sCb, long sCsplit, int want_splits, int* splits,
-                          hipStream_t st) {
+                          hipStream_t st, const GemmImp* imp, int imp_side) {
     if (splits) *splits = 0;
     if (M <= 0 || N <= 0 || batch <= 0) return 0;
     if (K <= 0 || !A || !B || !part || !splits) return JVAE_EINVAL;
@@ -510,6 +609,7 @@
     p.vecA = aligned16(A) && (sAb % 4 == 0) && (ak ? (sAm % 4 == 0) : (sAm == 1 && sAk % 4 == 0));
     p.vecB = aligned16(B) && (sBb % 4 == 0) && (bnc ? (sBk % 4 == 0) : (sBk == 1 && sBn % 4 == 0));
     *splits = splitk;
+    if (const int rc = set_imp(p, imp, imp_side, K)) return rc;
     if (gemm_x3_on(K)) return launch_x3(p, batch, st);
     return launch_tile<64, 64>(p, batch, st);
 }
diff --git a/joint-vae_amd/csrc/jvae_internal.h b/joint-vae_amd/csrc/jvae_internal.h
--- a/joint-vae_amd/csrc/jvae_internal.h
+++ b/joint-vae_amd/csrc/jvae_internal.h
@@ -1,17 +1,21 @@
 #pragma once
 #include <hip/hip_runtime.h>
+
+struct GemmImp;
 
 int jvae_gemm_launch(int M, int N, int K, int batch,
                      const float* A, long sAm, long sAk, long sAb,
                      const float* B, long sBk, long sBn, long sBb,
                      float* C, long sCm, long sCn, long sCb,
-                     const float* bias, int bias_mode, int flags, int splitk, hipStream_t st);
+                     const float* bias, int bias_mode, int flags, int splitk, hipStream_t st,
+                     const GemmImp* imp = nullptr, int imp_side = 0);
 
 int jvae_gemm_launch_ex(int M, int N, int K, int batch,
                         const float* A, long sAm, long sAk, long sAb,
                         const float* B, long sBk, long sBn, long sBb,
                         float* C, long sCm, long sCn, long sCb,
-                        const float* bias, int bias_mode, int bias_div, int flags, int splitk, hipStream_t st);
+                        const float* bias, int bias_mode, int bias_div, int flags, int splitk, hipStream_t st,
+                        const GemmImp* imp = nullptr, int imp_side = 0);
 
 int jvae_splitk_fold_qn(const float* part, const float* bias, float* y, int S, int N, int Cs, int Ps, hipStream_t st);
 int jvae_splitk_fold(const float* part, const float* bias, float* y, int S, long MN, int N, int relu, int accumulate,
@@ -21,7 +25,7 @@
                           const float* A, long sAm, long sAk, long sAb,
                           const float* B, long sBk, long sBn, long sBb,
                           float* part, long sCm, long sCn, long sCb, long sCsplit, int want_splits, int* splits,
-                          hipStream_t st);
+                          hipStream_t st, const GemmImp* imp = nullptr, int imp_side = 0);
 
 struct InAff { const float* sc; const float* sh; int relu; };
 
@@ -32,5 +36,15 @@
     int KH, KW, S, P;
 };
 
+struct GemmImp {
+    const float* x; const float* sc; const float* sh;
+    int act;
+    int Cb, Hb, Wb, KH, KW, KK, Ws, S, P, Nimg;
+    int rows;
+    unsigned mKK, mKW, mN, mWs;
+};
+constexpr int JVAE_GEMM_IMP_CH = 256;
+bool jvae_gemm_imp_make(const ConvGeom& g, const float* x, const InAff* aff, GemmImp* im);
+
 int jvae_wgrad_slab_reduce(const float* slab, float* dw, int G, int Ca, int Cb, int accumulate, int swapflip, hipStream_t st,
                            int tapmajor = 0, int taps = 25);
diff --git a/joint-vae_amd/jvae_hip/lib.py b/joint-vae_amd/jvae_hip/lib.py
--- a/joint-vae_amd/jvae_hip/lib.py
+++ b/joint-vae_amd/jvae_hip/lib.py
@@ -17,6 +17,7 @@
     'jvae_conv2d_workspace_bytes': (c_size_t, [c_int] * 11),
     'jvae_conv2d_set_split_bf16': (c_int, [c_int]),
     'jvae_conv2d_set_split_shape16': (c_int, [c_int]),
+    'jvae_conv2d_set_generic_implicit': (c_int, [c_int]),
     'jvae_conv2d_out_shape': (c_int, [c_int] * 8 + [POINTER(c_int), POINTER(c_int)]),
     'jvae_conv2d_route': (c_int, [c_int] * 17 + [POINTER(c_int), POINTER(c_int), POINTER(c_size_t), POINTER(c_int), POINTER(c_int)]),
     'jvae_conv2d_kernel_name': (c_char_p, [c_int]),
@@ -49,6 +50,7 @@
     'jvae_relu_bwd_b8': (c_int, [P, P, P, c_long, P]),
     'jvae_bn_finalize_f32': (c_int, [P] * 10 + [c_int, c_int, c_int, c_float, c_float, c_int, P, c_int, P, P, c_size_t, P]),
     'jvae_conv2d_affine_ok': (c_int, [c_int] * 11),
+    'jvae_conv2d_generic_affine_ok': (c_int, [c_int] * 11),
     'jvae_conv2d_fwd_aff_f32': (c_int, [P, P, P, P, P, POINTER(c_int), P, P, c_int] + [c_int] * 11 + [P, c_size_t, P]),
     'jvae_conv2d_wgrad_aff_f32': (c_int, [P, P, P, P, c_int, P, P, c_int] + [c_int] * 11 + [P, c_size_t, P]),
     'jvae_pack_cache_configure': (c_int, [P, c_size_t]),
diff --git a/joint-vae_amd/jvae_hip/ops.py b/joint-vae_amd/jvae_hip/ops.py
--- a/joint-vae_amd/jvae_hip/ops.py
+++ b/joint-vae_amd/jvae_hip/ops.py
@@ -212,6 +212,14 @@
     return bool(_geom_query('jvae_conv2d_affine_ok', spec.geom(N, H, W)))
 
 
+def conv_generic_affine_ok(spec, N, H, W):
+    return bool(L.load().jvae_conv2d_generic_affine_ok(*spec.geom(N, H, W)))
+
+
+def set_generic_implicit(on):
+    return L.load().jvae_conv2d_set_generic_implicit(int(on))
+
+
 ConvRoute = collections.namedtuple('ConvRoute', 'kernel swap ws splits aff_ok')
 ROUTE_DIR = {'fwd': 1, 'dgrad': 2, 'wgrad': 4}
 ROUTE_LAYOUT = {'f32': 0, 'b8': 1}
@@ -322,7 +330,7 @@
         return FWD | DGRAD | WGRAD
 
     def affine_ok(self, spec, N, H, W):
-        return conv_affine_ok(spec, N, H, W)
+        return conv_affine_ok(spec, N, H, W) or conv_generic_affine_ok(spec, N, H, W)
 
     def conv_fwd(self, x, w, b, spec, want_stats, aff, out_f32):
         if aff is not None:
```

Result: no change. 144,100 (-0.6%).
